# Genie-Kim/PintheMemory

Measured on AMD Instinct MI355X. Metric: train imgs/sec 768x768 bs=8 R50-DeepLabV3+ +mem, higher is better.
Workload: dtype f32

## Files before the change

### include/pinmem_hip.h

```cpp
#ifndef PINMEM_HIP_H
#define PINMEM_HIP_H
#include <stddef.h>
#include <stdint.h>

#ifdef __cplusplus
extern "C" {
#endif

typedef enum pm_status { PM_OK = 0, PM_EINVAL = -1, PM_EWORKSPACE = -2, PM_ELAUNCH = -3, PM_EUNSUPPORTED = -4 } pm_status;

typedef enum pm_dtype { PM_F32 = 0, PM_BF16 = 1 } pm_dtype;
#define PM_TF_ZERO_PAD64 1

typedef struct pm_tensor {
  void* ptr;
  int32_t n, h, w, c;
  int64_t pitch;
  int32_t dtype;
  int32_t flags;
} pm_tensor;

#define PM_ABI_VERSION 460

typedef struct pm_conv_params {
  int32_t struct_size;
  int32_t kh, kw, stride, pad, dil;
  int32_t prec;
  void* wino_v;
  int64_t wino_v_bytes;
  void* wxf;
  int64_t wxf_bytes;
  int32_t wxf_valid;
} pm_conv_params;

typedef struct pm_conv_epilogue {
  int64_t struct_size;
  const float* bias;
  const float* scale;
  const float* shift;
  const float* residual;
  int64_t residual_pitch;
  int32_t relu;
  float* bn_partials;
  int64_t bn_partials_bytes;
} pm_conv_epilogue;

const char* pm_last_error(void);
int pm_version(void);

size_t pm_conv_workspace(const pm_tensor* x, const pm_tensor* y, const pm_conv_params* p, int which );
size_t pm_conv_winograd_v_bytes(const pm_tensor* x, const pm_tensor* y, const pm_conv_params* p);
size_t pm_conv_wxf_bytes(const pm_tensor* x, const pm_tensor* y, const pm_conv_params* p);
size_t pm_conv_wxf_bytes_dgrad(const pm_tensor* dy, const pm_tensor* dx, const pm_conv_params* p);
typedef struct pm_wxf_job {
  const float* w;
  void* wxf;
  int64_t wxf_bytes;
  int32_t cout, kh, kw, cin;
  int32_t dgrad;
  int32_t reserved;
} pm_wxf_job;
int pm_conv_wxf_refresh_bf16(const pm_wxf_job* jobs, int n, void* stream);
int pm_conv_wxf_refresh_f32(const pm_wxf_job* jobs, int n, void* stream);
size_t pm_conv_bn_partials_bytes(const pm_tensor* x, const pm_tensor* y, const pm_conv_params* p);
int pm_conv_fwd(const pm_tensor* x, const float* w_krsc, const pm_tensor* y, const pm_conv_params* p,
                const pm_conv_epilogue* ep, void* ws, size_t ws_bytes, void* stream);
int pm_conv_bwd_data(const pm_tensor* dy, const float* w_krsc, const pm_tensor* dx, const pm_conv_params* p,
                     const pm_tensor* add, void* ws, size_t ws_bytes, void* stream);
int pm_conv_bwd_data_masked(const pm_tensor* dy, const float* w_krsc, const pm_tensor* dx, const pm_conv_params* p,
                            const pm_tensor* add, const uint8_t* add_mask, void* ws, size_t ws_bytes, void* stream);
int pm_conv_bwd_weight(const pm_tensor* x, const pm_tensor* dy, float* dw_krsc, float* dbias, const pm_conv_params* p,
                       void* ws, size_t ws_bytes, void* stream);

typedef struct pm_routing {
  int32_t struct_size;
  int32_t winograd;
  int32_t winograd_fused;
  int32_t conv16;
  int32_t conv16_wide;
  int32_t conv16_persistent;
  int32_t wgrad16;
  int32_t bf16_wgrad;
  int32_t split;
} pm_routing;
int pm_routing_get(pm_routing* out);
int pm_routing_set(const pm_routing* r);


int pm_set_winograd(int mode);
int pm_set_winograd_fused(int on);
int pm_set_conv16(int on);
int pm_set_bf16_wgrad(int on);
int pm_set_wgrad16(int on);
int pm_set_split(int on);

int pm_profile_enable(int on);
int pm_profile_dump(const char* csv_path);
int pm_profile_read(int mode, int bm, int bn, int km, int nst, double* total_ms, double* total_flops, int64_t* launches, int clear);
int pm_profile_read_prec(int mode, int bm, int bn, int km, int nst, int prec, double* total_ms, double* total_flops, int64_t* launches, int clear);
int pm_profile_read_bytes(int mode, int bm, int bn, int km, int nst, int prec, double* total_bytes);

size_t pm_bn_workspace(const pm_tensor* x);
int pm_bn_stats(const pm_tensor* x, float* moments, void* ws, size_t ws_bytes, void* stream);
int pm_bn_stats_finalize(const pm_tensor* x, float eps, float* mean, float* invstd, float* running_mean , float* running_var ,
                         float momentum, void* ws, size_t ws_bytes, void* stream);
int pm_bn_merge(const float* parts, int world, int c, float* moments, void* stream);
int pm_bn_merge_finalize(const float* parts, int world, int c, float eps, float* mean, float* invstd, float* running_mean ,
                         float* running_var , float momentum, void* stream);
int pm_bn_finalize(const float* moments, int c, float eps, float* mean, float* invstd,
                   float* running_mean, float* running_var, float momentum, void* stream);
int pm_bn_apply(const pm_tensor* x, const float* mean, const float* invstd, const float* gamma, const float* beta,
                const pm_tensor* residual , int relu, const pm_tensor* y, void* stream);
int pm_bn_apply_mask(const pm_tensor* x, const float* mean, const float* invstd, const float* gamma, const float* beta,
                     const pm_tensor* residual , int relu, const pm_tensor* y, uint8_t* mask , void* stream);
int pm_bn_bwd_reduce_mask(const pm_tensor* dy, const uint8_t* mask, const pm_tensor* x, const float* mean, const float* invstd,
                          const pm_tensor* gmask , float* sums, void* ws, size_t ws_bytes, void* stream);
int pm_bn_apply_mask_affine(const pm_tensor* x, const float* mean, const float* invstd, const float* gamma, const float* beta,
                            const pm_tensor* r, const float* r_mean, const float* r_invstd, const float* r_gamma, const float* r_beta,
                            int relu, const pm_tensor* y, uint8_t* mask , void* stream);
int pm_bn_bwd_apply_mask(const pm_tensor* dy, const uint8_t* mask, const pm_tensor* x, const float* mean, const float* invstd, const float* gamma,
                         const float* sums, float count, const pm_tensor* dx, void* stream);
int pm_bn_bwd_reduce(const pm_tensor* dy, const pm_tensor* y , const pm_tensor* x, const float* mean, const float* invstd,
                     const float* gamma , const float* beta , int relu, const pm_tensor* gmask ,
                     float* sums, void* ws, size_t ws_bytes, void* stream);
int pm_bn_bwd_apply(const pm_tensor* dy, const pm_tensor* y , const pm_tensor* x, const float* mean, const float* invstd,
                    const float* gamma, const float* beta , const float* sums, float count, int relu, const pm_tensor* dx,
                    const pm_tensor* dres , void* stream);
int pm_bn_partials_finalize(const float* partials, int64_t pixels, int c, float eps, float* mean, float* invstd, float* running_mean ,
                            float* running_var , float momentum, float* moments , void* stream);
int pm_bn_fold(const float* gamma, const float* beta, const float* running_mean, const float* running_var, const float* conv_bias,
               int c, float eps, float* scale, float* shift, void* stream);
int pm_bn_fold_multi(const void* table, const int* cs, const int* offs, int n, int max_c, int total, float eps, float* arena, void* stream);
int pm_relu_bwd(const pm_tensor* dy, const pm_tensor* y, const pm_tensor* dx, void* stream);
int pm_add(const pm_tensor* a, const pm_tensor* b, const pm_tensor* y, void* stream);
int pm_add_n(const pm_tensor* const* xs, int n, const pm_tensor* y, void* stream);
int pm_copy(const pm_tensor* src, const pm_tensor* dst, void* stream);
int pm_scale_shift_act(const pm_tensor* x, const float* scale, const float* shift, const pm_tensor* residual, int relu,
                       const pm_tensor* y, void* stream);

size_t pm_instnorm_workspace(int n, int h, int w, int c);
int pm_instnorm_fwd(const void* x, void* y, int n, int h, int w, int c, int64_t x_pitch, int64_t y_pitch, int dtype, const float* gamma ,
                    const float* beta , float eps, int relu, float* mean, float* invstd, void* ws, size_t ws_bytes, void* stream);
int pm_instnorm_bwd(const void* dy, const void* x, const void* y , void* dx, int n, int h, int w, int c, int64_t dy_pitch, int64_t x_pitch, int64_t y_pitch,
                    int64_t dx_pitch, int dtype, const float* gamma , const float* mean, const float* invstd, int relu, float* dgamma ,
                    float* dbeta , void* ws, size_t ws_bytes, void* stream);

int pm_cast(const pm_tensor* x, const pm_tensor* y, void* stream);

int pm_maxpool3x3s2_fwd(const pm_tensor* x, const pm_tensor* y, uint8_t* argmax, void* stream);
int pm_maxpool3x3s2_bwd(const pm_tensor* dy, const uint8_t* argmax, const pm_tensor* dx, void* stream);
int pm_maxpool3x3s2_bn_relu_fwd(const pm_tensor* x, const float* mean, const float* invstd, const float* gamma, const float* beta, const pm_tensor* y,
                                uint8_t* argmax, void* stream);
int pm_bn_bwd_reduce_pool(const pm_tensor* dy_pooled, const uint8_t* argmax, const pm_tensor* x, const float* mean, const float* invstd, const float* gamma,
                          const float* beta, float* sums, void* ws, size_t ws_bytes, void* stream);
int pm_bn_bwd_apply_pool(const pm_tensor* dy_pooled, const uint8_t* argmax, const pm_tensor* x, const float* mean, const float* invstd, const float* gamma,
// ... 176 lines not shown
```

### pinthememory_amd/csrc/conv_igemm.hip

```cpp
#include <stdlib.h>
#include <algorithm>
#include <type_traits>
#include <vector>

#include "pm_common.h"

#include "conv_igemm_kernel.h"

namespace {

template <int ZL, bool O16 = false>
__global__ __launch_bounds__(256) void splitk_reduce_vec_kernel(const float* __restrict__ ws, int ksplit, long slab, int M, int Nn,
                                                                float* __restrict__ C, long c_pitch, const float* bias,
                                                                const float* scale, const float* shift, const float* residual,
                                                                long res_pitch, int relu, const unsigned char* res_mask) {
  constexpr int GP = 256 / ZL;
  __shared__ float4 red[ZL > 1 ? ZL : 1][GP];
  const int gl = threadIdx.x % GP, zl = threadIdx.x / GP;
  const long groups = (long)M * Nn / 4;
  for (long g0 = (long)blockIdx.x * GP; g0 < groups; g0 += (long)gridDim.x * GP) {
    const long grp = g0 + gl;
    float4 v = make_float4(0.f, 0.f, 0.f, 0.f);
    if (grp < groups)
#pragma unroll 8
// ... 401 lines not shown
    return launch<MODE>(k, pl, st, 1, flops);
  });
}

int check_common(const pm_tensor* x, const pm_tensor* y, const pm_conv_params* p) {
  PM_REQUIRE(x && y && p && x->ptr && y->ptr, PM_EINVAL, "conv: null tensor");
  PM_REQUIRE(p->struct_size == (int32_t)sizeof(pm_conv_params), PM_EINVAL, "conv: pm_conv_params.struct_size %d != %zu -- caller built against another pinmem_hip.h (library ABI %d)",
             p->struct_size, sizeof(pm_conv_params), PM_ABI_VERSION);
  PM_REQUIRE(p->kh >= 1 && p->kw >= 1 && p->dil >= 1 && p->pad >= 0, PM_EINVAL, "conv: bad geometry");
  PM_REQUIRE(p->stride == 1 || p->stride == 2, PM_EUNSUPPORTED, "conv: stride %d unsupported (1 or 2)", p->stride);
  const int ho = (x->h + 2 * p->pad - p->dil * (p->kh - 1) - 1) / p->stride + 1;
  const int wo = (x->w + 2 * p->pad - p->dil * (p->kw - 1) - 1) / p->stride + 1;
  PM_REQUIRE(ho == y->h && wo == y->w && x->n == y->n, PM_EINVAL, "conv: output %dx%d does not match geometry (%dx%d)", y->h, y->w, ho, wo);
  PM_REQUIRE((x->dtype == PM_F32 || x->dtype == PM_BF16) && (y->dtype == PM_F32 || y->dtype == PM_BF16), PM_EUNSUPPORTED, "conv: dtype %d / %d", x->dtype, y->dtype);
  for (const pm_tensor* t : {x, y}) {
    if (pm_is_bf16(t)) PM_REQUIRE(pm_vec8(t), PM_EINVAL, "conv: bf16 tensors must be 16B aligned with pitch %% 8 == 0 and channels %% 8 == 0");
    else PM_REQUIRE(pm_vec_ok(t), PM_EINVAL, "conv: tensors must be 16B aligned with pitch %% 4 == 0");
  }
  PM_REQUIRE(x->c % 4 == 0, PM_EUNSUPPORTED, "conv: Cin %% 4 != 0 unsupported (pad the input channels)");
  PM_REQUIRE((y->c % 4 == 0) || (p->kh * p->kw == 1), PM_EUNSUPPORTED, "conv: Cout %% 4 != 0 only for 1x1");
  PM_REQUIRE(x->pitch >= x->c && y->pitch >= y->c, PM_EINVAL, "conv: pitch < channels");
  PM_REQUIRE(pm_pixels(x) * x->pitch < (1ll << 29) && pm_pixels(y) * y->pitch < (1ll << 29) && (int64_t)y->c * x->c * p->kh * p->kw < (1ll << 29),
             PM_EUNSUPPORTED, "conv: tensor too large for 32-bit byte offsets (2 GiB per tensor)");
  return PM_OK;
}

void fill_geom(ConvK& k, const pm_tensor* x, const pm_tensor* y, const pm_conv_params* p) {
  k.N = x->n, k.H = x->h, k.W = x->w, k.Cin = x->c, k.x_pitch = x->pitch;
  k.Ho = y->h, k.Wo = y->w, k.Cout = y->c, k.y_pitch = y->pitch;
  k.kh = p->kh, k.kw = p->kw, k.stride = p->stride, k.pad = p->pad, k.dil = p->dil;
  k.sshift = p->stride == 2 ? 1 : 0;
  k.prec = p->prec != 0 ? 1 : 0;
  k.T_eff = p->kh * p->kw, k.tk_w = p->kw, k.ky0 = k.kx0 = 0, k.ksy = k.ksx = 1;
  k.sub = k.sub_cy = k.sub_cx = 0, k.Hc = x->h, k.Wc = x->w;
  k.bias = k.scale = k.shift = k.residual = nullptr;
  k.res_pitch = 0, k.res_mask = nullptr, k.relu = 0, k.stats = nullptr, k.io16 = 0;
  k.stage_ep = 1;
  k.spl_prio = 1;
  k.n_group = 8;
  k.batch_xcd = 0;
  k.a_bs = k.b_bs = k.c_bs = 0;
}

struct WinoPlan {
  bool use;
  pm_wino_geom g;
  int Kp, P;
  size_t v_bytes, m_bytes, u_bytes;
  Plan pl;
};
inline bool wino_wgrad_pays(int cin, int cout) { return (long)cin * cout >= 256 * 256; }
WinoPlan wino_plan(const pm_tensor* xin, int cout, const pm_conv_params* p, bool wgrad = false) {
  WinoPlan wp{};
  if (wgrad && !wino_wgrad_pays(xin->c, cout)) return wp;
  if (pm_route.winograd == 0 || p->kh != 3 || p->kw != 3 || p->stride != 1 || p->pad != p->dil || p->prec != 0) return wp;
  const int cin = xin->c;
  if (cin < 128 || cout < 128 || (cout & 3) || (cin & 3)) return wp;
  int m = 0;
  double best_ratio = 0.6;
  for (int cand = pm_route.winograd; cand >= 2; cand -= 2) {
    const pm_wino_geom g = pm_wino_make_geom(xin->n, xin->h, xin->w, p->dil, cand);
    const double cover = (double)(cand * g.TY * p->dil) * (double)(cand * g.TX * p->dil) / ((double)xin->h * xin->w);
    const double ratio = cover * (cand + 2) * (cand + 2) / (9.0 * cand * cand);
    if (ratio <= best_ratio) best_ratio = ratio, m = cand, wp.g = g;
  }
  if (!m) return wp;
  wp.P = (m + 2) * (m + 2);
  wp.Kp = (cin + BK - 1) / BK * BK;
  if (wp.g.tiles * (long)std::max(wp.Kp, cout) * 4 >= (1ll << 31)) return wp;
  wp.v_bytes = pm_align_up((size_t)wp.P * wp.g.tiles * wp.Kp * sizeof(float), 256);
  wp.m_bytes = pm_align_up((size_t)wp.P * wp.g.tiles * cout * sizeof(float), 256);
  wp.u_bytes = pm_align_up((size_t)wp.P * cout * wp.Kp * sizeof(float), 256);
  wp.pl.bm = 128, wp.pl.bn = 128;
  if (pm_cdiv(cout, 128) * 128 > cout * 1.12 && pm_cdiv(cout, 64) * 64 < pm_cdiv(cout, 128) * 128) wp.pl.bn = 64;
  if (wp.g.tiles <= 4608 && !pm_route.split) wp.pl.bm = 64;
  wp.pl.tiles_m = pm_cdiv(wp.g.tiles, wp.pl.bm), wp.pl.tiles_n = pm_cdiv(cout, wp.pl.bn);
  wp.pl.ksplit = 1, wp.pl.kper = wp.Kp, wp.pl.ws_bytes = 0;
  wp.use = true;
  return wp;
}
inline size_t wino_ws(const WinoPlan& wp) { return wp.v_bytes + wp.m_bytes + wp.u_bytes; }

int wino_conv(const pm_tensor* xin, const float* w, int w_cout, int w_cin, bool dgrad, const pm_tensor* yout, const WinoPlan& wp,
              const pm_conv_epilogue& ep, void* ws, hipStream_t st, float* v_keep = nullptr, float* u_ext = nullptr, bool u_valid = false) {
  float* V = v_keep ? v_keep : (float*)ws;
  float* Mo = (float*)((char*)ws + wp.v_bytes);
  float* U = u_ext ? u_ext : (float*)((char*)ws + wp.v_bytes + wp.m_bytes);
  const int cout = yout->c;
  if (int e = pm_wino_input_xf((const float*)xin->ptr, xin->pitch, xin->c, wp.Kp, wp.g, V, st)) return e;
  if (!(u_ext && u_valid))
    if (int e = pm_wino_filter_xf(w, w_cout, w_cin, wp.Kp, dgrad, wp.g.m, U, st)) return e;
  const pm_tensor xv = {V, 1, 1, (int32_t)wp.g.tiles, wp.Kp, wp.Kp};
  const pm_tensor yv = {Mo, 1, 1, (int32_t)wp.g.tiles, cout, cout};
  const pm_conv_params p1 = {(int32_t)sizeof(pm_conv_params), 1, 1, 1, 0, 1, 0};
  ConvK k;
  fill_geom(k, &xv, &yv, &p1);
  k.A = V, k.B = U, k.C = Mo;
  k.M = (int)wp.g.tiles, k.Nn = cout, k.K = wp.Kp;
  k.a_bytes = (unsigned)(wp.g.tiles * wp.Kp * 4), k.b_bytes = (unsigned)((long)cout * wp.Kp * 4), k.kmode = K_FAST;
  k.c_pitch = cout, k.c_split = 0;
  k.a_bs = wp.g.tiles * wp.Kp, k.b_bs = (long)cout * wp.Kp, k.c_bs = wp.g.tiles * cout;
  if (pm_route.winograd_fused && wp.g.m == 4 && wp.Kp % 16 == 0) {
    ProfScope prof(st, 3, 32, 32, 0, 0, 1, wp.g.tiles, cout, wp.Kp, wp.P, 1, 2.0 * wp.P * (double)wp.g.tiles * cout * xin->c);
    const int e = pm_wino_fused_f4(V, U, cout, wp.Kp, wp.g, (float*)yout->ptr, yout->pitch, ep.bias, ep.scale, ep.shift, ep.residual, ep.residual_pitch, ep.relu, st);
    prof.done();
    return e;
  }
  if (int e = launch<MODE_FWD>(k, wp.pl, st, wp.P, 2.0 * wp.P * (double)wp.g.tiles * cout * xin->c)) return e;
  return pm_wino_output_xf(Mo, cout, wp.g, (float*)yout->ptr, yout->pitch, ep.bias, ep.scale, ep.shift, ep.residual, ep.residual_pitch, ep.relu, st);
}

struct WinoWgradPlan {
  Plan pl;
  size_t slab_bytes;
};
WinoWgradPlan wino_wgrad_plan(const WinoPlan& wp, int cout) {
  WinoWgradPlan q{};
  q.pl.bm = 128, q.pl.bn = 128;
  if (pm_cdiv(wp.Kp, 128) * 128 > wp.Kp * 1.12 && pm_cdiv(wp.Kp, 64) * 64 < pm_cdiv(wp.Kp, 128) * 128) q.pl.bn = 64;
  q.pl.tiles_m = pm_cdiv(cout, 128), q.pl.tiles_n = pm_cdiv(wp.Kp, q.pl.bn);
  const long ksteps = (wp.g.tiles + BK - 1) / BK;
  const long per_split = (long)q.pl.tiles_m * q.pl.tiles_n * wp.P;
  long ks = std::max<long>(1, std::min<long>((768 + per_split / 2) / per_split, ksteps / 8));
  const long steps_per = (ksteps + ks - 1) / ks;
  ks = (ksteps + steps_per - 1) / steps_per;
  q.pl.ksplit = (int)ks, q.pl.kper = (int)(steps_per * BK), q.pl.ws_bytes = 0;
  q.slab_bytes = pm_align_up((size_t)ks * wp.P * cout * wp.Kp * sizeof(float), 256);
  return q;
}
inline size_t wino_wgrad_ws(const WinoPlan& wp, const WinoWgradPlan& q) { return wp.v_bytes + wp.m_bytes + q.slab_bytes; }

int wino_wgrad(const pm_tensor* x, const pm_tensor* dy, float* dw, const WinoPlan& wp, const WinoWgradPlan& q, void* ws, hipStream_t st,
               float* v_kept = nullptr) {
  float* V = v_kept ? v_kept : (float*)ws;
  float* Z = (float*)((char*)ws + wp.v_bytes);
  float* slab = (float*)((char*)ws + wp.v_bytes + wp.m_bytes);
  const int cout = dy->c;
  if (!v_kept)
    if (int e = pm_wino_input_xf((const float*)x->ptr, x->pitch, x->c, wp.Kp, wp.g, V, st)) return e;
  if (int e = pm_wino_dy_xf((const float*)dy->ptr, dy->pitch, cout, wp.g, Z, st)) return e;
  const pm_tensor xv = {V, 1, 1, (int32_t)wp.g.tiles, wp.Kp, wp.Kp};
  const pm_tensor zv = {Z, 1, 1, (int32_t)wp.g.tiles, cout, cout};
  const pm_conv_params p1 = {(int32_t)sizeof(pm_conv_params), 1, 1, 1, 0, 1, 0};
  ConvK k;
  fill_geom(k, &xv, &zv, &p1);
  k.A = Z, k.B = V, k.C = slab;
  k.M = cout, k.Nn = wp.Kp, k.K = (int)wp.g.tiles;
  k.a_bytes = (unsigned)(wp.g.tiles * cout * 4), k.b_bytes = (unsigned)(wp.g.tiles * wp.Kp * 4), k.kmode = K_MID;
  k.c_pitch = wp.Kp, k.c_split = (long)wp.P * cout * wp.Kp;
  k.a_bs = wp.g.tiles * cout, k.b_bs = wp.g.tiles * wp.Kp, k.c_bs = (long)cout * wp.Kp;
  if (int e = launch<MODE_WGRAD>(k, q.pl, st, wp.P, 2.0 * wp.P * (double)wp.g.tiles * cout * x->c)) return e;
  return pm_wino_dw_xf(slab, q.pl.ksplit, cout, x->c, wp.Kp, wp.g.m, dw, st);
}

struct Bf16Plan {
  bool use;
  bool c16;
  pm_conv16 k16;
  bool inplace;
  int Cp;
  long M, Nn, Kf;
  size_t xb_bytes, wb_bytes;
  Plan pl;
};
Bf16Plan bf16_plan(const pm_tensor* xin, const pm_tensor* yout, const pm_conv_params* p) {
  Bf16Plan b{};
  if ((p->prec != 2 && !pm_is_bf16(xin) && !pm_is_bf16(yout)) || xin->c < 32) return b;
  b.Cp = (xin->c + 63) / 64 * 64;
  const long T = (long)p->kh * p->kw;
  b.M = pm_pixels(yout), b.Nn = yout->c, b.Kf = T * b.Cp / 2;
  b.inplace = pm_is_bf16(xin) && (xin->c % 64 == 0 || ((xin->flags & PM_TF_ZERO_PAD64) && xin->pitch >= b.Cp));
  const size_t xb = b.inplace ? (size_t)pm_pixels(xin) * xin->pitch * 2 : (size_t)pm_pixels(xin) * b.Cp * 2, wb = (size_t)yout->c * T * b.Cp * 2;
  if (xb >= (1ull << 31) || wb >= (1ull << 31)) return b;
  b.xb_bytes = b.inplace ? 0 : pm_align_up(xb, 256), b.wb_bytes = pm_align_up(wb, 256);
  b.pl = make_plan(MODE_FWD, b.M, b.Nn, b.Kf, true);
  if (b.pl.bn < 64) return b;
  b.use = true;
  constexpr long C16_MIN_M = 256;
  b.c16 = false;
  if (pm_route.conv16 && b.M >= C16_MIN_M && p->stride >= 1) {
    pm_conv16& k = b.k16;
    k = pm_conv16{};
    k.N = xin->n, k.H = xin->h, k.W = xin->w, k.Ho = yout->h, k.Wo = yout->w;
    k.a_pitch = b.inplace ? xin->pitch : b.Cp, k.Cp = b.Cp;
    k.kh = p->kh, k.kw = p->kw, k.stride = p->stride, k.pad = p->pad, k.dil = p->dil;
    k.M = (int)b.M, k.Nn = (int)b.Nn, k.K = (int)(T * b.Cp), k.ksteps = k.K / 64;
    k.c_pitch = yout->pitch, k.c_f32 = pm_is_bf16(yout) ? 0 : 1;
    pm_conv16_plan(&k);
    b.c16 = pm_route.conv16 == 2 || k.wide || k.bm == 64 || k.ksteps_per == 1 || (b.pl.bm == 64 && k.ksteps >= 16);
  }
  return b;
}
inline size_t bf16_ws(const Bf16Plan& b) {
  return b.xb_bytes + b.wb_bytes + std::max(pm_align_up(b.pl.ws_bytes, 256), b.c16 ? pm_conv16_slab_bytes(&b.k16) : (size_t)0);
}

int conv_bf16(const pm_tensor* xin, const float* w, int w_cout, int w_cin, bool rotate, const pm_tensor* yout, const pm_conv_params* pe, const Bf16Plan& b,
              const pm_conv_epilogue& e0, void* ws, hipStream_t st, char* wb_ext = nullptr, bool wb_valid = false) {
  char* xb = b.inplace ? (char*)xin->ptr : (char*)ws;
  char* wb = wb_ext ? wb_ext : (char*)ws + b.xb_bytes;
  float* slab = (float*)((char*)ws + b.xb_bytes + b.wb_bytes);
  const int T = pe->kh * pe->kw;
  if (!b.inplace) {
    if (pm_is_bf16(xin)) {
      if (int e = pm16_pad_rows((const pm_bf16*)xin->ptr, xin->pitch, xin->c, b.Cp, pm_pixels(xin), (pm_bf16*)xb, st)) return e;
    } else if (int e = pm_bf16_cast_rows((const float*)xin->ptr, xin->pitch, xin->c, b.Cp, pm_pixels(xin), xb, st)) return e;
  }
  if (!(wb_ext && wb_valid))
    if (int e = pm_bf16_cast_weights(w, w_cout, T, w_cin, b.Cp, rotate, wb, st)) return e;
  const long xpitch16 = b.inplace ? xin->pitch : b.Cp;
  if (b.c16) {
    const bool o16 = pm_is_bf16(yout);
    const bool ok = (!e0.bn_partials || o16) &&
                    (o16 ? ((yout->c | yout->pitch | (e0.residual ? e0.residual_pitch : 0)) & 7) == 0 && pm_aligned16(yout->ptr) && pm_aligned16(e0.residual)
                         : !(e0.scale || e0.residual || e0.relu));
    if (ok) {
      pm_conv16 k = b.k16;
      k.A = (const pm_bf16*)xb, k.B = (const pm_bf16*)wb;
      const double fl = 2.0 * (double)b.M * (double)b.Nn * (double)T * (double)xin->c * (g_prof_on ? pm_conv16_executed_fraction(&k) : 1.0);
      ProfScope prof(st, k.wide ? 5 : 4, k.bm, k.bn, pm_conv16w_persistent(&k), 5, k.wide ? 3 : (k.ksteps_per == 1 ? 1 : 2), k.M, k.Nn, k.K / 2, 1, k.ksplit, fl);
      return run_planned(k.ksplit, b.M, b.Nn, slab, (float*)yout->ptr, (long)yout->pitch, e0, o16, nullptr, st, [&](float* C, bool slabs) {
        k.C = C;
        if (!slabs) set_epilogue(k, e0), k.stats = o16 ? e0.bn_partials : nullptr;
// ... 407 lines not shown
}
extern "C" int pm_set_split(int on) {
  pm_route.split = on ? 1 : 0;
  return PM_OK;
}
extern "C" int pm_set_bf16_wgrad(int on) {
  pm_route.bf16_wgrad = on != 0;
  return PM_OK;
}
extern "C" int pm_profile_enable(int on) {
  g_prof_on = on != 0;
  return PM_OK;
}
extern "C" int pm_profile_read_prec(int mode, int bm, int bn, int km, int nst, int prec, double* total_ms, double* total_flops, int64_t* launches, int clear);
extern "C" int pm_profile_read(int mode, int bm, int bn, int km, int nst, double* total_ms, double* total_flops, int64_t* launches, int clear) {
  return pm_profile_read_prec(mode, bm, bn, km, nst, -1, total_ms, total_flops, launches, clear);
}
extern "C" int pm_profile_read_prec(int mode, int bm, int bn, int km, int nst, int prec, double* total_ms, double* total_flops, int64_t* launches, int clear) {
  double ms = 0.0, fl = 0.0;
  int64_t n = 0;
  for (const ProfRec& r : g_prof) {
    if ((mode >= 0 && r.mode != mode) || (bm >= 0 && r.bm != bm) || (bn >= 0 && r.bn != bn) || (km >= 0 && r.km != km) || (nst >= 0 && r.nst != nst) ||
        (prec >= 0 && r.prec != prec))
      continue;
    float t = 0.f;
    if (hipEventSynchronize(r.b) != hipSuccess || hipEventElapsedTime(&t, r.a, r.b) != hipSuccess) continue;
    ms += t, fl += r.flops, ++n;
  }
  if (clear) {
    for (const ProfRec& r : g_prof) (void)hipEventDestroy(r.a), (void)hipEventDestroy(r.b);
    g_prof.clear();
  }
  if (total_ms) *total_ms = ms;
  if (total_flops) *total_flops = fl;
  if (launches) *launches = n;
  return PM_OK;
}

extern "C" int pm_profile_read_bytes(int mode, int bm, int bn, int km, int nst, int prec, double* total_bytes) {
  double b = 0.0;
  for (const ProfRec& r : g_prof) {
    if ((mode >= 0 && r.mode != mode) || (bm >= 0 && r.bm != bm) || (bn >= 0 && r.bn != bn) || (km >= 0 && r.km != km) || (nst >= 0 && r.nst != nst) ||
        (prec >= 0 && r.prec != prec))
      continue;
    b += r.bytes;
  }
  if (total_bytes) *total_bytes = b;
  return PM_OK;
}

extern "C" int pm_profile_dump(const char* path) {
  PM_REQUIRE(path, PM_EINVAL, "pm_profile_dump: null path");
  FILE* f = fopen(path, "w");
  PM_REQUIRE(f, PM_EINVAL, "pm_profile_dump: cannot open %s", path);
  fprintf(f, "mode,bm,bn,km,nst,prec,M,N,K,batch,ksplit,ms,gflop\n");
  for (const ProfRec& r : g_prof) {
    float t = 0.f;
    if (hipEventSynchronize(r.b) != hipSuccess || hipEventElapsedTime(&t, r.a, r.b) != hipSuccess) continue;
    fprintf(f, "%d,%d,%d,%d,%d,%d,%d,%d,%d,%d,%d,%.5f,%.4f\n", r.mode, r.bm, r.bn, r.km, r.nst, r.prec, r.M, r.Nn, r.K, r.batch, r.ksplit, t, r.flops * 1e-9);
  }
  fclose(f);
  return PM_OK;
}

extern "C" size_t pm_conv_workspace(const pm_tensor* x, const pm_tensor* y, const pm_conv_params* p0, int which) {
  const pm_conv_params tp = tier_params(p0, x, y);
  return route_conv(which, x, y, &tp).ws_bytes;
}
extern "C" size_t pm_conv_winograd_v_bytes(const pm_tensor* x, const pm_tensor* y, const pm_conv_params* p0) {
  if (!x || !y || !p0) return 0;
  const pm_conv_params tp = tier_params(p0, x, y);
  return route_conv(MODE_FWD, x, y, &tp).v_keep_bytes;
}
extern "C" size_t pm_conv_wxf_bytes(const pm_tensor* x, const pm_tensor* y, const pm_conv_params* p0) {
  if (!x || !y || !p0) return 0;
  const pm_conv_params tp = tier_params(p0, x, y);
  return route_conv(MODE_FWD, x, y, &tp).wxf_bytes;
}
extern "C" size_t pm_conv_wxf_bytes_dgrad(const pm_tensor* dy, const pm_tensor* dx, const pm_conv_params* p0) {
  if (!dy || !dx || !p0) return 0;
  const pm_conv_params tp = tier_params(p0, dy, dx);
  return route_conv(MODE_DGRAD, dx, dy, &tp).wxf_bytes;
}
extern "C" size_t pm_conv_bn_partials_bytes(const pm_tensor* x, const pm_tensor* y, const pm_conv_params* p0) {
  if (!x || !y || !p0 || check_common(x, y, p0) != PM_OK) return 0;
  const pm_conv_params tp = tier_params(p0, x, y);
  return route_conv(MODE_FWD, x, y, &tp).bn_bytes;
}

extern "C" int pm_conv_wxf_refresh_f32(const pm_wxf_job* jobs, int n, void* stream) {
  PM_REQUIRE(n >= 0 && (jobs || n == 0), PM_EINVAL, "conv_wxf_refresh_f32: bad job table");
  std::vector<const float*> w(n);
  std::vector<float*> U(n);
  std::vector<int> cout(n), cin(n), kp(n), m(n);
  for (int i = 0; i < n; ++i) {
    const pm_wxf_job& q = jobs[i];
    PM_REQUIRE(q.w && q.wxf && q.cout > 0 && q.cin > 0 && q.kh == 3 && q.kw == 3 && q.dgrad == 0, PM_EINVAL,
               "conv_wxf_refresh_f32: job %d: forward transforms of 3x3 filters only", i);
    PM_REQUIRE(pm_aligned16(q.wxf), PM_EINVAL, "conv_wxf_refresh_f32: job %d: buffer must be 16-byte aligned", i);
    const int Kp = (q.cin + BK - 1) / BK * BK;
    const size_t u4 = pm_align_up((size_t)36 * q.cout * Kp * sizeof(float), 256), u2 = pm_align_up((size_t)16 * q.cout * Kp * sizeof(float), 256);
    PM_REQUIRE((size_t)q.wxf_bytes == u4 || (size_t)q.wxf_bytes == u2, PM_EINVAL, "conv_wxf_refresh_f32: job %d: %ld bytes is neither the F(4x4) nor the F(2x2) transform of %d x %d",
               i, (long)q.wxf_bytes, q.cout, q.cin);
    w[i] = q.w, U[i] = (float*)q.wxf, cout[i] = q.cout, cin[i] = q.cin, kp[i] = Kp, m[i] = (size_t)q.wxf_bytes == u4 ? 4 : 2;
  }
  return pm_wino_filter_xf_multi(w.data(), U.data(), cout.data(), cin.data(), kp.data(), m.data(), n, (hipStream_t)stream);
}

extern "C" int pm_conv_fwd(const pm_tensor* x, const float* w, const pm_tensor* y, const pm_conv_params* p0,
                           const pm_conv_epilogue* ep, void* ws, size_t ws_bytes, void* stream) {
  if (int e = check_common(x, y, p0)) return e;
  const pm_conv_params tp = tier_params(p0, x, y);
  const pm_conv_params* p = &tp;
  PM_REQUIRE(!ep || ep->struct_size == (int64_t)sizeof(pm_conv_epilogue), PM_EINVAL,
             "conv_fwd: pm_conv_epilogue.struct_size %ld != %zu -- caller built against another pinmem_hip.h (library ABI %d)", ep ? (long)ep->struct_size : 0l,
             sizeof(pm_conv_epilogue), PM_ABI_VERSION);
  PM_REQUIRE(w && pm_aligned16(w), PM_EINVAL, "conv_fwd: weight null or unaligned");
  pm_conv_epilogue e0 = {(int64_t)sizeof(pm_conv_epilogue), nullptr, nullptr, nullptr, nullptr, 0, 0};
  if (ep) e0 = *ep;
  PM_REQUIRE((e0.scale == nullptr) == (e0.shift == nullptr), PM_EINVAL, "conv_fwd: scale and shift go together");
  const ConvRoute r = route_conv(MODE_FWD, x, y, p);
  if (e0.bn_partials) {
    PM_REQUIRE(!e0.relu && !e0.residual, PM_EINVAL, "conv_fwd: bn_partials are the statistics of the convolution output (no residual / ReLU)");
    PM_REQUIRE(r.bn_bytes != 0 && (size_t)e0.bn_partials_bytes >= r.bn_bytes, PM_EINVAL, "conv_fwd: this call cannot emit bn_partials (ask pm_conv_bn_partials_bytes): %zu needed", r.bn_bytes);
  }
  PM_REQUIRE(ws_bytes >= r.ws_bytes && (ws || r.ws_bytes == 0), PM_EWORKSPACE, "conv_fwd: workspace %zu < %zu", ws_bytes, r.ws_bytes);
  hipStream_t st = (hipStream_t)stream;
  switch (r.kind) {
    case R_WINO: {
      float* keep = (p->wino_v && (size_t)p->wino_v_bytes >= r.wino.v_bytes) ? (float*)p->wino_v : nullptr;
      float* uext = (p->wxf && (size_t)p->wxf_bytes >= r.wino.u_bytes) ? (float*)p->wxf : nullptr;
      return wino_conv(x, w, y->c, x->c, false, y, r.wino, e0, ws, st, keep, uext, p->wxf_valid != 0);
    }
    case R_BF16: {
      char* wext = (p->wxf && (size_t)p->wxf_bytes >= r.b16.wb_bytes) ? (char*)p->wxf : nullptr;
      return conv_bf16(x, w, y->c, x->c, false, y, &r.pe, r.b16, e0, ws, st, wext, p->wxf_valid != 0);
    }
    default:
      PM_REQUIRE(pm_is_f32(x), PM_EUNSUPPORTED, "conv_fwd: a bf16 input needs at least 32 channels (got %d)", x->c);
      return conv_direct<MODE_FWD>(x, y, w, p, r.pl, e0, ws, st);
  }
}

extern "C" int pm_conv_bwd_data(const pm_tensor* dy, const float* w, const pm_tensor* dx, const pm_conv_params* p0, const pm_tensor* add,
                                void* ws, size_t ws_bytes, void* stream) {
  return pm_conv_bwd_data_masked(dy, w, dx, p0, add, nullptr, ws, ws_bytes, stream);
}

extern "C" int pm_conv_bwd_data_masked(const pm_tensor* dy, const float* w, const pm_tensor* dx, const pm_conv_params* p0, const pm_tensor* add,
                                       const uint8_t* add_mask, void* ws, size_t ws_bytes, void* stream) {
  if (int e = check_common(dx, dy, p0)) return e;
  const pm_conv_params tp = tier_params(p0, dy, dx);
  const pm_conv_params* p = &tp;
  PM_REQUIRE(!add || (add->ptr && pm_same_shape(add, dx) && add->dtype == dx->dtype), PM_EINVAL, "conv_bwd_data: `add` must match dx (shape and dtype)");
  PM_REQUIRE(!add || !pm_is_bf16(add) || pm_vec8(add), PM_EINVAL, "conv_bwd_data: bf16 `add` must be 16B aligned with pitch %% 8 == 0");
  PM_REQUIRE(w && pm_aligned16(w), PM_EINVAL, "conv_bwd_data: weight null or unaligned");
  const ConvRoute r = route_conv(MODE_DGRAD, dx, dy, p);
  PM_REQUIRE(ws_bytes >= r.ws_bytes && (ws || r.ws_bytes == 0), PM_EWORKSPACE, "conv_bwd_data: workspace %zu < %zu", ws_bytes, r.ws_bytes);
  if (add_mask) {
    PM_REQUIRE(add && pm_is_f32(add) && pm_is_f32(dy) && pm_vec4(add) && pm_vec4(dx), PM_EINVAL, "conv_bwd_data: a masked `add` is an fp32 tensor with 16-byte rows and c %% 4 == 0");
    PM_REQUIRE(r.kind == R_DIRECT, PM_EUNSUPPORTED,
               "conv_bwd_data: a masked `add` is served by the fp32 implicit-GEMM route only (this call routes to %s)",
               r.kind == R_WINO ? "Winograd" : (r.kind == R_BF16 ? "the bf16 kernels" : "the stride-2 class kernels"));
  }
  hipStream_t st = (hipStream_t)stream;
  const pm_conv_epilogue e1 = {(int64_t)sizeof(pm_conv_epilogue), nullptr, nullptr, nullptr, add ? (const float*)add->ptr : nullptr, add ? add->pitch : 0, 0};
  switch (r.kind) {
    case R_S2_NATIVE: return dgrad_s2_bf16(dy, w, dx, p, add, r.s2n, ws, st);
    case R_S2_PARITY: return dgrad_s2_parity(dy, w, dx, p, add, r, ws, st);
    case R_BF16: {
      char* wext = (p->wxf && (size_t)p->wxf_bytes >= r.b16.wb_bytes) ? (char*)p->wxf : nullptr;
      return conv_bf16(dy, w, dy->c, dx->c, true, dx, &r.pe, r.b16, e1, ws, st, wext, p->wxf_valid != 0);
    }
    case R_WINO: return wino_conv(dy, w, dy->c, dx->c, true, dx, r.wino, e1, ws, st);
    default:
      PM_REQUIRE(pm_is_f32(dy), PM_EUNSUPPORTED, "conv_bwd_data: a bf16 dy needs at least 32 channels and a stride-1 geometry the forward form covers");
      return conv_direct<MODE_DGRAD>(dx, dy, w, p, r.pl, e1, ws, st, add_mask);
  }
}

extern "C" int pm_conv_bwd_weight(const pm_tensor* x0, const pm_tensor* dy0, float* dw, float* dbias, const pm_conv_params* p0, void* ws,
                                  size_t ws_bytes, void* stream) {
  if (int e = check_common(x0, dy0, p0)) return e;
  const pm_conv_params tp = tier_params(p0, x0, dy0);
  const pm_conv_params* p = &tp;
  PM_REQUIRE(dw && pm_aligned16(dw), PM_EINVAL, "conv_bwd_weight: dw null or unaligned");
  const ConvRoute r = route_conv(MODE_WGRAD, x0, dy0, p);
  PM_REQUIRE(ws && ws_bytes >= r.ws_bytes, PM_EWORKSPACE, "conv_bwd_weight: workspace %zu < %zu", ws_bytes, r.ws_bytes);
  hipStream_t st = (hipStream_t)stream;
  const pm_tensor *x = x0, *dy = dy0;
  pm_tensor x32, dy32;
  if (!r.native16 && pm_is_bf16(x0)) {
    if (int e = upcast(x0, (char*)ws + r.x32_off, &x32, st)) return e;
    x = &x32;
  }
  if (pm_is_bf16(dy0) && (!r.native16 || dbias)) {
    if (int e = upcast(dy0, (char*)ws + r.dy32_off, &dy32, st)) return e;
    if (!r.native16) dy = &dy32;
  }
  int e;
  switch (r.kind) {
    case R_BF16_WGRAD: e = conv_wgrad_bf16(x, dy, dw, p, r.b16w, ws, st); break;
    case R_WINO_WGRAD: e = wino_wgrad(x, dy, dw, r.wino, r.wino_w, ws, st, (p->wino_v && (size_t)p->wino_v_bytes >= r.wino.v_bytes) ? (float*)p->wino_v : nullptr); break;
    default: e = conv_wgrad_direct(x, dy, dw, p, r, ws, st);
  }
  if (e || !dbias) return e;
  const pm_tensor* dyb = pm_is_bf16(dy0) ? &dy32 : dy0;
  const long P = pm_pixels(dyb);
  const int rpb = colsum_rows(P, dyb->c), nb = pm_cdiv(P, rpb);
  float* part = (float*)((char*)ws + r.bias_off);
  if (dyb->pitch == ((dyb->c + 3) & ~3) && dyb->pitch <= 64 && pm_aligned16(dyb->ptr))
    hipLaunchKernelGGL(colsum_partial_narrow_kernel, dim3(nb), dim3(256), 0, st, (const float*)dyb->ptr, (int)(dyb->pitch / 4), P, dyb->c, rpb, part);
  else
    hipLaunchKernelGGL(colsum_partial_kernel, dim3(nb, pm_cdiv(dyb->c, 64)), dim3(256), 0, st, (const float*)dyb->ptr, (long)dyb->pitch, P, dyb->c, rpb, part);
  hipLaunchKernelGGL(colsum_final_kernel, dim3(pm_cdiv(dyb->c, 64)), dim3(1024), 0, st, (const float*)part, nb, dyb->c, dbias);
  return pm_check_launch("conv_bias_grad");
}
```

### pinthememory_amd/csrc/pm_common.h

```cpp
#pragma once
#include <hip/hip_runtime.h>
#include <algorithm>
#include <atomic>
#include <stdarg.h>
#include <stdint.h>
#include <stdio.h>

#include "../../include/pinmem_hip.h"

void pm_set_error(const char* fmt, ...);

#define PM_REQUIRE(cond, code, ...)      \
  do {                                   \
    if (!(cond)) {                       \
      pm_set_error(__VA_ARGS__);         \
      return (code);                     \
    }                                    \
  } while (0)

static inline int pm_check_launch(const char* what) {
  hipError_t e = hipGetLastError();
  if (e != hipSuccess) {
    pm_set_error("%s: launch failed: %s", what, hipGetErrorString(e));
    return PM_ELAUNCH;
  }
  return PM_OK;
}

static inline bool pm_aligned16(const void* p) { return (reinterpret_cast<uintptr_t>(p) & 15u) == 0; }
static inline int64_t pm_pixels(const pm_tensor* t) { return (int64_t)t->n * t->h * t->w; }
static inline int pm_cdiv(int64_t a, int64_t b) { return (int)((a + b - 1) / b); }
static inline size_t pm_align_up(size_t v, size_t a) { return (v + a - 1) / a * a; }

static inline bool pm_vec_ok(const pm_tensor* t) { return pm_aligned16(t->ptr) && (t->pitch % 4) == 0; }
static inline bool pm_is_f32(const pm_tensor* t) { return t->dtype == PM_F32; }
static inline bool pm_is_bf16(const pm_tensor* t) { return t->dtype == PM_BF16; }
#define PM_REQUIRE_F32(t, who) PM_REQUIRE(!(t) || pm_is_f32(t), PM_EUNSUPPORTED, "%s: fp32 tensors only (got dtype %d)", who, (t)->dtype)
static inline bool pm_vec8(const pm_tensor* t) { return pm_is_bf16(t) && pm_aligned16(t->ptr) && (t->pitch % 8) == 0 && (t->c % 8) == 0; }

struct pm_wino_geom {
  int N, H, W, d, m, TY, TX;
  long tiles;
};
pm_wino_geom pm_wino_make_geom(int n, int h, int w, int d, int m);
int pm_wino_input_xf(const float* x, long pitch, int C, int Kp, const pm_wino_geom& g, float* V, hipStream_t st);
int pm_wino_filter_xf(const float* w, int Cout, int Cin, int Kp, bool dgrad, int m, float* U, hipStream_t st);
int pm_wino_filter_xf_multi(const float* const* w, float* const* U, const int* cout, const int* cin, const int* kp, const int* m, int n, hipStream_t st);
int pm_wino_output_xf(const float* M, int Cout, const pm_wino_geom& g, float* y, long ypitch, const float* bias, const float* scale, const float* shift,
                      const float* residual, long res_pitch, int relu, hipStream_t st);
int pm_wino_fused_f4(const float* V, const float* U, int Cout, int Kp, const pm_wino_geom& g, float* y, long ypitch, const float* bias, const float* scale,
                     const float* shift, const float* residual, long res_pitch, int relu, hipStream_t st);
int pm_wino_dy_xf(const float* dy, long pitch, int Cout, const pm_wino_geom& g, float* Z, hipStream_t st);
int pm_wino_dw_xf(const float* slab, int ks, int Cout, int Cin, int Kp, int m, float* dw, hipStream_t st);

int pm_bf16_cast_rows(const float* x, long pitch, int C, int Cp, long P, void* out, hipStream_t st);
int pm_bf16_cast_weights(const float* w, int Cout, int T, int Cin, int Cp, bool rotate, void* out, hipStream_t st);
struct PmS2Classes {
  int ky0[4], nky[4], kx0[4], nkx[4];
  void* out[4];
};
int pm_bf16_cast_weights_s2(const float* w, int Cout, int kh, int kw, int Cin, int Cp, const PmS2Classes* cl, hipStream_t st);
int pm_bf16_transpose_taps(const float* x, long pitch, int C, int N, int H, int W, int Ho, int Wo, int kh, int kw, int stride, int pad, int dil, void* out,
                           hipStream_t st);

typedef unsigned short pm_bf16;
int pm16_to_f32(const pm_bf16* x, long pitch, int C, long P, float* out, long out_pitch, hipStream_t st);
int pm16_pad_rows(const pm_bf16* x, long pitch, int C, int Cp, long P, pm_bf16* out, hipStream_t st);

struct pm_conv16 {
  const pm_bf16* A;
  const pm_bf16* B;
  void* C;
  int N, H, W, Ho, Wo;
  long a_pitch;
  int Cp;
  int kh, kw, stride, pad, dil;
  int M, Nn, K, ksteps;
  long c_pitch;
  int c_f32;
  const float *bias, *scale, *shift;
  const void* residual;
  long res_pitch;
  int relu;
  float* stats;
  int bm, bn, tiles_m, tiles_n, ksplit, ksteps_per;
  long c_split;
  int wide;
};
void pm_conv16_plan(pm_conv16* k);
int pm_conv16w_launch(const pm_conv16* k, hipStream_t st);
int pm_conv16w_persistent(const pm_conv16* k);
size_t pm_conv16_slab_bytes(const pm_conv16* k);
double pm_conv16_executed_fraction(const pm_conv16* k);
int pm_conv16_launch(const pm_conv16* k, hipStream_t st);

struct pm_wgrad16 {
  const pm_bf16* X;
  const pm_bf16* DY;
  float* C;
  int N, H, W, Ho, Wo;
  long x_pitch, dy_pitch;
  int Cin, Cout, kh, kw, stride, pad, dil;
  int M, Nn, P;
  int kper, ksplit;
  long c_split;
  int bm, bn, tiles_m, tiles_n;
};
bool pm_wgrad16_plan(pm_wgrad16* k);
int pm_wgrad16_launch(const pm_wgrad16* k, hipStream_t st);

struct pm_gemm_pw {
  const float* A;
  const float* B;
  float* C;
  const float *bias, *scale, *shift, *residual;
  const unsigned char* res_mask;
  long a_pitch, c_pitch, res_pitch;
  int b_sn, b_sk;
  long M;
  int Nn, K, relu;
};
bool pm_pwstream_ok(const pm_gemm_pw* g);
int pm_pwstream_launch(const pm_gemm_pw* g, hipStream_t st);

constexpr int PM_MAX_DEVICES = 64;
inline int pm_device_cus(int dev) {
  static std::atomic<int> cached[PM_MAX_DEVICES];
  const bool keep = dev >= 0 && dev < PM_MAX_DEVICES;
// ... 307 lines not shown
```

### pinthememory_amd/csrc/winograd.hip

```cpp
#include "pm_common.h"

namespace {

enum { W_BT = 0, W_AT = 1, W_G = 2, W_A = 3, W_GT = 4 };

template <int MT>
__host__ __device__ constexpr float wino_bt(int i, int j) {
  if (MT == 2) {
    constexpr float t[4][4] = {{1, 0, -1, 0}, {0, 1, 1, 0}, {0, -1, 1, 0}, {0, 1, 0, -1}};
    return t[i & 3][j & 3];
  }
  constexpr float t[6][6] = {{4, 0, -5, 0, 1, 0}, {0, -4, -4, 1, 1, 0}, {0, 4, -4, -1, 1, 0}, {0, -2, -1, 2, 1, 0}, {0, 2, -1, -2, 1, 0}, {0, 4, 0, -5, 0, 1}};
  return t[i][j];
}
template <int MT>
__host__ __device__ constexpr float wino_at(int i, int j) {
  if (MT == 2) {
    constexpr float t[2][4] = {{1, 1, 1, 0}, {0, 1, -1, -1}};
    return t[i & 1][j & 3];
  }
  constexpr float t[4][6] = {{1, 1, 1, 1, 1, 0}, {0, 1, -1, 2, -2, 0}, {0, 1, 1, 4, 4, 0}, {0, 1, -1, 8, -8, 1}};
  return t[i][j];
}
template <int MT>
// ... 2 lines not shown
    constexpr float t[4][3] = {{1, 0, 0}, {0.5f, 0.5f, 0.5f}, {0.5f, -0.5f, 0.5f}, {0, 0, 1}};
    return t[i & 3][j];
  }
  constexpr float t[6][3] = {{1.f / 4, 0, 0},          {-1.f / 6, -1.f / 6, -1.f / 6}, {-1.f / 6, 1.f / 6, -1.f / 6},
                             {1.f / 24, 1.f / 12, 1.f / 6}, {1.f / 24, -1.f / 12, 1.f / 6},  {0, 0, 1}};
  return t[i][j];
}
template <int MT, int WHICH>
__host__ __device__ constexpr float wino_coef(int r, int c) {
  return WHICH == W_BT ? wino_bt<MT>(r, c) : WHICH == W_AT ? wino_at<MT>(r, c) : WHICH == W_G ? wino_g<MT>(r, c) : WHICH == W_A ? wino_at<MT>(c, r) : wino_g<MT>(c, r);
}

template <int W>
struct Vec {
  float v[W];
};
template <int W>
__device__ __forceinline__ Vec<W> vzero() {
  Vec<W> r;
#pragma unroll
  for (int i = 0; i < W; ++i) r.v[i] = 0.f;
  return r;
}
template <int W>
__device__ __forceinline__ Vec<W> vload(const float* p) {
  Vec<W> r;
  if constexpr (W == 4) {
    const float4 q = PM_LD4(p);
    r.v[0] = q.x, r.v[1] = q.y, r.v[2] = q.z, r.v[3] = q.w;
  } else if constexpr (W == 2) {
    const float2 q = *reinterpret_cast<const float2*>(p);
    r.v[0] = q.x, r.v[1] = q.y;
  } else {
    r.v[0] = *p;
  }
  return r;
}
template <int W>
__device__ __forceinline__ void vstore(float* p, const Vec<W>& r) {
  if constexpr (W == 4) PM_ST4(p, make_float4(r.v[0], r.v[1], r.v[2], r.v[3]));
  else if constexpr (W == 2) *reinterpret_cast<float2*>(p) = make_float2(r.v[0], r.v[1]);
  else *p = r.v[0];
}

template <int MT, int WHICH, int R, int C, int W>
__device__ __forceinline__ void mat_apply(const Vec<W> (&in)[C], Vec<W> (&out)[R]) {
#pragma unroll
  for (int r = 0; r < R; ++r) {
    Vec<W> acc = vzero<W>();
    bool first = true;
#pragma unroll
    for (int c = 0; c < C; ++c) {
      const float k = wino_coef<MT, WHICH>(r, c);
      if (k == 0.f) continue;
#pragma unroll
      for (int i = 0; i < W; ++i) {
        if (first) acc.v[i] = k == 1.f ? in[c].v[i] : (k == -1.f ? -in[c].v[i] : k * in[c].v[i]);
        else if (k == 1.f) acc.v[i] += in[c].v[i];
        else if (k == -1.f) acc.v[i] -= in[c].v[i];
        else acc.v[i] = fmaf(k, in[c].v[i], acc.v[i]);
      }
      first = false;
    }
    out[r] = acc;
  }
}

struct TileId {
  int n, ry, rx, ty, tx;
};
__device__ __forceinline__ TileId decode_tile(unsigned tile, const pm_wino_geom& g) {
  TileId t;
  t.tx = (int)(tile % (unsigned)g.TX);
  unsigned q = tile / (unsigned)g.TX;
  t.ty = (int)(q % (unsigned)g.TY);
  q /= (unsigned)g.TY;
  t.rx = (int)(q % (unsigned)g.d);
  q /= (unsigned)g.d;
  t.ry = (int)(q % (unsigned)g.d);
  t.n = (int)(q / (unsigned)g.d);
  return t;
}

template <int MT, int W>
__global__ __launch_bounds__(256) void wino_input_kernel(const float* __restrict__ x, long xp, int C, int Kp, const pm_wino_geom g, float* __restrict__ V) {
  constexpr int A = MT + 2;
  const unsigned kg = Kp / W;
  const unsigned total = (unsigned)g.tiles * kg;
  const long plane = g.tiles * (long)Kp;
  for (unsigned i = blockIdx.x * 256u + threadIdx.x; i < total; i += gridDim.x * 256u) {
    const unsigned tile = i / kg;
    const int c = (int)(i - tile * kg) * W;
    const TileId t = decode_tile(tile, g);
    const bool cok = c < C;
    Vec<W> tt[A][A];
#pragma unroll
    for (int b = 0; b < A; ++b) {
      const int xx = t.rx + g.d * (MT * t.tx + b - 1);
      const bool xok = cok && (unsigned)xx < (unsigned)g.W;
      Vec<W> col[A], o[A];
#pragma unroll
      for (int a = 0; a < A; ++a) {
        const int yy = t.ry + g.d * (MT * t.ty + a - 1);
        col[a] = (xok && (unsigned)yy < (unsigned)g.H) ? vload<W>(x + ((long)(t.n * g.H + yy) * g.W + xx) * xp + c) : vzero<W>();
      }
      mat_apply<MT, W_BT>(col, o);
#pragma unroll
      for (int a = 0; a < A; ++a) tt[a][b] = o[a];
    }
    float* out = V + (long)tile * Kp + c;
#pragma unroll
    for (int a = 0; a < A; ++a) {
      Vec<W> o[A];
      mat_apply<MT, W_BT>(tt[a], o);
#pragma unroll
      for (int b = 0; b < A; ++b) vstore<W>(out + (a * A + b) * plane, o[b]);
    }
  }
}

template <int MT, int W>
__global__ __launch_bounds__(256) void wino_output_kernel(const float* __restrict__ M, int Cout, const pm_wino_geom g, float* __restrict__ y, long yp,
                                                          const float* __restrict__ bias, const float* __restrict__ scale,
                                                          const float* __restrict__ shift, const float* __restrict__ residual, long rp, int relu) {
  constexpr int A = MT + 2;
  const unsigned cg = Cout / W;
  const unsigned total = (unsigned)g.tiles * cg;
  const long plane = g.tiles * (long)Cout;
  for (unsigned i = blockIdx.x * 256u + threadIdx.x; i < total; i += gridDim.x * 256u) {
    const unsigned tile = i / cg;
    const int c = (int)(i - tile * cg) * W;
    const TileId t = decode_tile(tile, g);
    const float* in = M + (long)tile * Cout + c;
    Vec<W> s[MT][A];
#pragma unroll
    for (int b = 0; b < A; ++b) {
      Vec<W> col[A], o[MT];
#pragma unroll
      for (int a = 0; a < A; ++a) col[a] = vload<W>(in + (a * A + b) * plane);
      mat_apply<MT, W_AT>(col, o);
#pragma unroll
      for (int a = 0; a < MT; ++a) s[a][b] = o[a];
    }
    Vec<W> bi = vzero<W>(), sc = vzero<W>(), sh = vzero<W>();
    if (bias) bi = vload<W>(bias + c);
    if (scale) sc = vload<W>(scale + c), sh = vload<W>(shift + c);
#pragma unroll
    for (int a = 0; a < MT; ++a) {
      const int yy = t.ry + g.d * (MT * t.ty + a);
      Vec<W> o[MT];
      mat_apply<MT, W_AT>(s[a], o);
#pragma unroll
      for (int b = 0; b < MT; ++b) {
        const int xx = t.rx + g.d * (MT * t.tx + b);
        if (yy >= g.H || xx >= g.W) continue;
        const long pix = (long)(t.n * g.H + yy) * g.W + xx;
        Vec<W> v = o[b];
        if (bias) {
#pragma unroll
          for (int q = 0; q < W; ++q) v.v[q] += bi.v[q];
        }
        if (scale) {
#pragma unroll
          for (int q = 0; q < W; ++q) v.v[q] = v.v[q] * sc.v[q] + sh.v[q];
        }
        if (residual) {
          const Vec<W> rr = vload<W>(residual + pix * rp + c);
#pragma unroll
          for (int q = 0; q < W; ++q) v.v[q] += rr.v[q];
        }
        if (relu) {
#pragma unroll
          for (int q = 0; q < W; ++q) v.v[q] = fmaxf(v.v[q], 0.f);
        }
        vstore<W>(y + pix * yp + c, v);
      }
    }
  }
}

template <int MT, bool DGRAD>
__device__ __forceinline__ void wino_filter_block(const float* __restrict__ w, int Cout, int Cin, int Kp, float* __restrict__ U, int bx, int by,
                                                  float (*sg)[32][33]) {
  constexpr int A = MT + 2;
  const int tx = threadIdx.x & 31, ty = threadIdx.x >> 5;
  const int R = DGRAD ? Cin : Cout;
  const int Kr = DGRAD ? Cout : Cin;
// ... 16 lines not shown
    Vec<4> col[3], o[A];
#pragma unroll
    for (int ky = 0; ky < 3; ++ky)
#pragma unroll
      for (int e = 0; e < 4; ++e) col[ky].v[e] = DGRAD ? sg[(2 - ky) * 3 + (2 - kx)][4 * q + e][j] : sg[ky * 3 + kx][j][4 * q + e];
    mat_apply<MT, W_G>(col, o);
#pragma unroll
    for (int a = 0; a < A; ++a) gg[a][kx] = o[a];
  }
  float* out = U + (long)row * Kp + k;
#pragma unroll
  for (int a = 0; a < A; ++a) {
    Vec<4> o[A];
    mat_apply<MT, W_G>(gg[a], o);
#pragma unroll
    for (int b = 0; b < A; ++b) {
#pragma unroll
      for (int e = 0; e < 4; ++e)
        if (k + e >= Kr) o[b].v[e] = 0.f;
      vstore<4>(out + (a * A + b) * plane, o[b]);
    }
  }
}
template <int MT, bool DGRAD>
__global__ __launch_bounds__(256) void wino_filter_kernel(const float* __restrict__ w, int Cout, int Cin, int Kp, float* __restrict__ U) {
  __shared__ float sg[9][32][33];
  wino_filter_block<MT, DGRAD>(w, Cout, Cin, Kp, U, blockIdx.x, blockIdx.y, sg);
}

constexpr int WR_BATCH = 48;
struct WinoRefreshJobs {
  const float* w[WR_BATCH];
  float* U[WR_BATCH];
  int cout[WR_BATCH], cin[WR_BATCH], kp[WR_BATCH], m[WR_BATCH];
  int start[WR_BATCH + 1];
  int n;
};
__global__ __launch_bounds__(256) void wino_filter_multi_kernel(const WinoRefreshJobs t) {
  __shared__ float sg[9][32][33];
  int j = 0;
  while (j + 1 < t.n && (int)blockIdx.x >= t.start[j + 1]) ++j;
  const int local = (int)blockIdx.x - t.start[j];
  const int nbx = t.kp[j] / 32;
  const int bx = local % nbx, by = local / nbx;
  if (t.m[j] == 4) wino_filter_block<4, false>(t.w[j], t.cout[j], t.cin[j], t.kp[j], t.U[j], bx, by, sg);
  else wino_filter_block<2, false>(t.w[j], t.cout[j], t.cin[j], t.kp[j], t.U[j], bx, by, sg);
}

template <int MT, int W>
__global__ __launch_bounds__(256) void wino_dy_kernel(const float* __restrict__ dy, long yp, int Cout, const pm_wino_geom g, float* __restrict__ Z) {
  constexpr int A = MT + 2;
  const unsigned cg = Cout / W;
  const unsigned total = (unsigned)g.tiles * cg;
  const long plane = g.tiles * (long)Cout;
  for (unsigned i = blockIdx.x * 256u + threadIdx.x; i < total; i += gridDim.x * 256u) {
    const unsigned tile = i / cg;
    const int c = (int)(i - tile * cg) * W;
    const TileId t = decode_tile(tile, g);
    Vec<W> r[A][MT];
#pragma unroll
    for (int b = 0; b < MT; ++b) {
      const int xx = t.rx + g.d * (MT * t.tx + b);
      Vec<W> col[MT], o[A];
#pragma unroll
      for (int a = 0; a < MT; ++a) {
        const int yy = t.ry + g.d * (MT * t.ty + a);
        col[a] = (yy < g.H && xx < g.W) ? vload<W>(dy + ((long)(t.n * g.H + yy) * g.W + xx) * yp + c) : vzero<W>();
      }
      mat_apply<MT, W_A>(col, o);
#pragma unroll
      for (int a = 0; a < A; ++a) r[a][b] = o[a];
    }
    float* out = Z + (long)tile * Cout + c;
#pragma unroll
    for (int a = 0; a < A; ++a) {
      Vec<W> o[A];
      mat_apply<MT, W_A>(r[a], o);
#pragma unroll
      for (int b = 0; b < A; ++b) vstore<W>(out + (a * A + b) * plane, o[b]);
    }
  }
}

template <int MT>
__global__ __launch_bounds__(256) void wino_dw_kernel(const float* __restrict__ slab, int ks, int Cout, int Cin, int Kp, float* __restrict__ dw) {
  constexpr int A = MT + 2, P = A * A;
  const long total = (long)Cout * Cin, plane = (long)Cout * Kp;
  for (long i = (long)blockIdx.x * 256 + threadIdx.x; i < total; i += (long)gridDim.x * 256) {
    const int co = (int)(i / Cin), ci = (int)(i - (long)co * Cin);
    const float* in = slab + (long)co * Kp + ci;
    float du[P];
#pragma unroll
    for (int q = 0; q < P; ++q) du[q] = 0.f;
    for (int z = 0; z < ks; ++z) {
      float ld[P];
#pragma unroll
      for (int q = 0; q < P; ++q) ld[q] = in[((long)z * P + q) * plane];
#pragma unroll
      for (int q = 0; q < P; ++q) du[q] += ld[q];
    }
    Vec<1> h[3][A];
#pragma unroll
    for (int b = 0; b < A; ++b) {
      Vec<1> col[A], o[3];
#pragma unroll
      for (int a = 0; a < A; ++a) col[a].v[0] = du[a * A + b];
      mat_apply<MT, W_GT>(col, o);
#pragma unroll
      for (int k = 0; k < 3; ++k) h[k][b] = o[k];
    }
    float* out = dw + (long)co * 9 * Cin + ci;
#pragma unroll
    for (int k = 0; k < 3; ++k) {
      Vec<1> o[3];
      mat_apply<MT, W_GT>(h[k], o);
#pragma unroll
      for (int l = 0; l < 3; ++l) out[(k * 3 + l) * (long)Cin] = o[l].v[0];
    }
  }
}

typedef float f32x16 __attribute__((ext_vector_type(16)));

struct WinoFusedArgs {
  const float* V;
  const float* U;
  float* y;
  long yp;
  int Cout, Kp;
  pm_wino_geom g;
  const float* bias;
  const float* scale;
  const float* shift;
  const float* residual;
  long rp;
  int relu;
  int ncb;
};

constexpr int WF_THREADS = 768, WF_TB = 32, WF_CB = 32, WF_BK = 16, WF_P = 36;
constexpr size_t WF_LDS = (size_t)WF_P * WF_TB * (WF_CB + 1) * sizeof(float);

__global__ __launch_bounds__(WF_THREADS) void wino_fused_f4_kernel(const WinoFusedArgs a) {
  extern __shared__ __align__(16) float4 lds4[];
  const int tid = threadIdx.x, lane = tid & 63, wave = tid >> 6;
  const int lid = pm_xcd_remap(blockIdx.x, gridDim.x);
  const int tb = lid / a.ncb, cb = lid - tb * a.ncb;
  const long tile0 = (long)tb * WF_TB;
  const int co0 = cb * WF_CB;

  const int rem = tid & 255, row = rem >> 2, chunk = rem & 3, pgrp = tid >> 8;
  const bool is_a = row < WF_TB;
  bool valid;
  const float* gp;
  long plane;
  if (is_a) {
    const long tile = tile0 + row;
    valid = tile < a.g.tiles;
    gp = a.V + (valid ? tile : 0) * a.Kp + chunk * 4;
    plane = a.g.tiles * (long)a.Kp;
  } else {
    const int co = co0 + row - WF_TB;
    valid = co < a.Cout;
    gp = a.U + (long)(valid ? co : 0) * a.Kp + chunk * 4;
    plane = (long)a.Cout * a.Kp;
  }
// ... 29 lines not shown
      acc[j] = __builtin_amdgcn_mfma_f32_32x32x2f32(a0.z, b0.z, acc[j], 0, 0, 0);
      acc[j] = __builtin_amdgcn_mfma_f32_32x32x2f32(a0.w, b0.w, acc[j], 0, 0, 0);
      acc[j] = __builtin_amdgcn_mfma_f32_32x32x2f32(a1.x, b1.x, acc[j], 0, 0, 0);
      acc[j] = __builtin_amdgcn_mfma_f32_32x32x2f32(a1.y, b1.y, acc[j], 0, 0, 0);
      acc[j] = __builtin_amdgcn_mfma_f32_32x32x2f32(a1.z, b1.z, acc[j], 0, 0, 0);
      acc[j] = __builtin_amdgcn_mfma_f32_32x32x2f32(a1.w, b1.w, acc[j], 0, 0, 0);
    }
  };

  const int nk = a.Kp / WF_BK;
  gload(0);
  lstore();
  __syncthreads();
  for (int kt = 0; kt < nk; ++kt) {
    if (kt + 1 < nk) gload((kt + 1) * WF_BK);
    compute();
    __syncthreads();
    if (kt + 1 < nk) {
      lstore();
      __syncthreads();
    }
  }

  float* Ms = reinterpret_cast<float*>(lds4);
#pragma unroll
  for (int j = 0; j < 3; ++j) {
    const int pnt = wave * 3 + j;
#pragma unroll
    for (int q = 0; q < 16; ++q) Ms[(pnt * WF_TB + (q & 3) + 8 * (q >> 2) + 4 * half) * (WF_CB + 1) + l31] = acc[j][q];
  }
  __syncthreads();
  constexpr int MT = 4, A = 6;
  for (int idx = tid; idx < WF_TB * WF_CB; idx += WF_THREADS) {
    const int t = idx >> 5, c = idx & 31;
    const long tile = tile0 + t;
    const int co = co0 + c;
    if (tile >= a.g.tiles || co >= a.Cout) continue;
    const TileId ti = decode_tile((unsigned)tile, a.g);
    Vec<1> sv[MT][A];
#pragma unroll
    for (int b = 0; b < A; ++b) {
      Vec<1> col[A], o[MT];
#pragma unroll
      for (int aa = 0; aa < A; ++aa) col[aa].v[0] = Ms[((aa * A + b) * WF_TB + t) * (WF_CB + 1) + c];
      mat_apply<MT, W_AT>(col, o);
#pragma unroll
      for (int aa = 0; aa < MT; ++aa) sv[aa][b] = o[aa];
    }
    const float bi = a.bias ? a.bias[co] : 0.f, sc = a.scale ? a.scale[co] : 0.f, sh = a.scale ? a.shift[co] : 0.f;
#pragma unroll
    for (int aa = 0; aa < MT; ++aa) {
      const int yy = ti.ry + a.g.d * (MT * ti.ty + aa);
      Vec<1> o[MT];
      mat_apply<MT, W_AT>(sv[aa], o);
#pragma unroll
      for (int b = 0; b < MT; ++b) {
        const int xx = ti.rx + a.g.d * (MT * ti.tx + b);
        if (yy >= a.g.H || xx >= a.g.W) continue;
        const long pix = (long)(ti.n * a.g.H + yy) * a.g.W + xx;
        float v = o[b].v[0];
        if (a.bias) v += bi;
        if (a.scale) v = v * sc + sh;
        if (a.residual) v += a.residual[pix * a.rp + co];
        if (a.relu) v = fmaxf(v, 0.f);
        a.y[pix * a.yp + co] = v;
      }
    }
  }
}

inline unsigned nblocks(long total) { return (unsigned)std::min<long>((total + 255) / 256, 1 << 20); }

}

pm_wino_geom pm_wino_make_geom(int n, int h, int w, int d, int m) {
  pm_wino_geom g;
  g.N = n, g.H = h, g.W = w, g.d = d, g.m = m;
  g.TY = (pm_cdiv(h, d) + m - 1) / m, g.TX = (pm_cdiv(w, d) + m - 1) / m;
  g.tiles = (long)n * d * d * g.TY * g.TX;
  return g;
}

int pm_wino_input_xf(const float* x, long pitch, int C, int Kp, const pm_wino_geom& g, float* V, hipStream_t st) {
  if (g.m == 4) hipLaunchKernelGGL((wino_input_kernel<4, 2>), dim3(nblocks(g.tiles * (Kp / 2))), dim3(256), 0, st, x, pitch, C, Kp, g, V);
  else hipLaunchKernelGGL((wino_input_kernel<2, 4>), dim3(nblocks(g.tiles * (Kp / 4))), dim3(256), 0, st, x, pitch, C, Kp, g, V);
  return pm_check_launch("wino_input");
}

int pm_wino_filter_xf(const float* w, int Cout, int Cin, int Kp, bool dgrad, int m, float* U, hipStream_t st) {
  const int R = dgrad ? Cin : Cout;
  dim3 grid(Kp / 32, pm_cdiv(R, 32));
  if (m == 4) {
    if (dgrad) hipLaunchKernelGGL((wino_filter_kernel<4, true>), grid, dim3(256), 0, st, w, Cout, Cin, Kp, U);
    else hipLaunchKernelGGL((wino_filter_kernel<4, false>), grid, dim3(256), 0, st, w, Cout, Cin, Kp, U);
  } else {
    if (dgrad) hipLaunchKernelGGL((wino_filter_kernel<2, true>), grid, dim3(256), 0, st, w, Cout, Cin, Kp, U);
    else hipLaunchKernelGGL((wino_filter_kernel<2, false>), grid, dim3(256), 0, st, w, Cout, Cin, Kp, U);
  }
  return pm_check_launch("wino_filter");
}

int pm_wino_filter_xf_multi(const float* const* w, float* const* U, const int* cout, const int* cin, const int* kp, const int* m, int n, hipStream_t st) {
  for (int i0 = 0; i0 < n; i0 += WR_BATCH) {
    WinoRefreshJobs t;
    t.n = std::min(WR_BATCH, n - i0);
    long blocks = 0;
    for (int i = 0; i < t.n; ++i) {
      t.w[i] = w[i0 + i], t.U[i] = U[i0 + i], t.cout[i] = cout[i0 + i], t.cin[i] = cin[i0 + i], t.kp[i] = kp[i0 + i], t.m[i] = m[i0 + i];
      t.start[i] = (int)blocks;
      blocks += (long)(kp[i0 + i] / 32) * pm_cdiv(cout[i0 + i], 32);
    }
    t.start[t.n] = (int)blocks;
    if (blocks == 0) continue;
    hipLaunchKernelGGL(wino_filter_multi_kernel, dim3((unsigned)blocks), dim3(256), 0, st, t);
    if (int e = pm_check_launch("wino_filter_multi")) return e;
  }
  return PM_OK;
}

int pm_wino_output_xf(const float* M, int Cout, const pm_wino_geom& g, float* y, long ypitch, const float* bias, const float* scale, const float* shift,
                      const float* residual, long res_pitch, int relu, hipStream_t st) {
  if (g.m == 4)
    hipLaunchKernelGGL((wino_output_kernel<4, 2>), dim3(nblocks(g.tiles * (Cout / 2))), dim3(256), 0, st, M, Cout, g, y, ypitch, bias, scale, shift, residual,
                       res_pitch, relu);
  else
    hipLaunchKernelGGL((wino_output_kernel<2, 4>), dim3(nblocks(g.tiles * (Cout / 4))), dim3(256), 0, st, M, Cout, g, y, ypitch, bias, scale, shift, residual,
                       res_pitch, relu);
  return pm_check_launch("wino_output");
}

int pm_wino_dy_xf(const float* dy, long pitch, int Cout, const pm_wino_geom& g, float* Z, hipStream_t st) {
  if (g.m == 4) hipLaunchKernelGGL((wino_dy_kernel<4, 2>), dim3(nblocks(g.tiles * (Cout / 2))), dim3(256), 0, st, dy, pitch, Cout, g, Z);
  else hipLaunchKernelGGL((wino_dy_kernel<2, 4>), dim3(nblocks(g.tiles * (Cout / 4))), dim3(256), 0, st, dy, pitch, Cout, g, Z);
  return pm_check_launch("wino_dy");
}

int pm_wino_dw_xf(const float* slab, int ks, int Cout, int Cin, int Kp, int m, float* dw, hipStream_t st) {
  const unsigned nb = (unsigned)std::min<long>(((long)Cout * Cin + 255) / 256, 1 << 16);
  if (m == 4) hipLaunchKernelGGL(wino_dw_kernel<4>, dim3(nb), dim3(256), 0, st, slab, ks, Cout, Cin, Kp, dw);
  else hipLaunchKernelGGL(wino_dw_kernel<2>, dim3(nb), dim3(256), 0, st, slab, ks, Cout, Cin, Kp, dw);
  return pm_check_launch("wino_dw");
}

int pm_wino_fused_f4(const float* V, const float* U, int Cout, int Kp, const pm_wino_geom& g, float* y, long ypitch, const float* bias, const float* scale,
                     const float* shift, const float* residual, long res_pitch, int relu, hipStream_t st) {
  static pm_lds_optin optin;
  (void)optin(reinterpret_cast<const void*>(&wino_fused_f4_kernel), (int)WF_LDS);
  WinoFusedArgs a;
  a.V = V, a.U = U, a.y = y, a.yp = ypitch, a.Cout = Cout, a.Kp = Kp, a.g = g;
  a.bias = bias, a.scale = scale, a.shift = shift, a.residual = residual, a.rp = res_pitch, a.relu = relu;
  a.ncb = (Cout + WF_CB - 1) / WF_CB;
  const long ntb = (g.tiles + WF_TB - 1) / WF_TB;
  hipLaunchKernelGGL(wino_fused_f4_kernel, dim3((unsigned)(ntb * a.ncb)), dim3(WF_THREADS), WF_LDS, st, a);
  return pm_check_launch("wino_fused_f4");
}
```

### pinthememory_amd/hip/kernels.py

```python
import ctypes
from ctypes import byref

import os
import weakref

import torch

from . import lib as L
from .lib import PmConvEpilogue, PmConvParams, check, ptr, stream, tdesc, workspace


def _lib():
    return L.load()


CONV_PREC = 0
ACT_DTYPE = torch.float32


def set_conv_precision(name):
    global CONV_PREC, ACT_DTYPE
    CONV_PREC = {'f32': 0, 'fp32': 0, 'bf16': 2, 'bf16_operands': 2, 'bf16_staged': 1}[name]
    ACT_DTYPE = torch.bfloat16 if name == 'bf16' else torch.float32

# ... 128 lines not shown
            self.nbytes += nbu
        else:
            del self[key]
        self[key] = ent
        ent.used = True
        version = owner._version
        valid = ent.version == version
        if not valid:
            ent.version = -1
        p.wxf, p.wxf_bytes, p.wxf_valid = ent.buf.data_ptr(), nbu, 1 if valid else 0
        raw, cur = self._stream()
        if valid and ent.event is not None and ent.stream != raw:
            cur.wait_event(ent.event)
        return None if valid else (ent, version)

    def commit(self, *pending):
        raw, cur = self._stream()
        event = cur.record_event()
        for ent, version in pending:
            ent.version, ent.event, ent.stream = version, event, raw

    def forget_events(self):
        for ent in self.values():
            ent.event = ent.stream = None


_U_CACHE = _FilterCache()
clear_filters, forget_filter_events = _U_CACHE.clear, _U_CACHE.forget_events

_REFRESH = {2: ('pm_conv_wxf_refresh_bf16', False), 0: ('pm_conv_wxf_refresh_f32', True)}


def refresh_filters():
    if KEEP_WINOGRAD_U is False or not _U_CACHE or CONV_PREC not in _REFRESH:
        return 0
    entry_point, forward_3x3_only = _REFRESH[CONV_PREC]
    dev = torch.cuda.current_device()
    todo = []
    for ent in _U_CACHE.values():
        if ent.prec != CONV_PREC or ent.device != dev or not ent.used:
            continue
        cout, kh, kw, cin = ent.shape
        if forward_3x3_only and (ent.dgrad or kh != 3 or kw != 3):
            continue
        ent.used = False
        owner = ent.owner()
        if owner is None or owner.data_ptr() != ent.ptr or ent.version == owner._version or not ent.buf.is_cuda:
            continue
        todo.append((ent, owner._version))
    if not todo:
        return 0
    jobs = (L.PmWxfJob * len(todo))()
    for j, (ent, version) in zip(jobs, todo):
        cout, kh, kw, cin = ent.shape
        j.w, j.wxf, j.wxf_bytes, j.cout, j.kh, j.kw, j.cin, j.dgrad = ent.ptr, ent.buf.data_ptr(), ent.nbytes, cout, kh, kw, cin, 1 if ent.dgrad else 0
        ent.version = -1
    check(getattr(_lib(), entry_point)(jobs, len(todo), stream()), entry_point)
    _U_CACHE.commit(*todo)
    return len(todo)


_SIZES = {}
_GEN = [0]


def _sizes(key, fn):
    v = _SIZES.get(key)
    if v is None:
        if len(_SIZES) > 8192:
            _SIZES.clear()
        v = _SIZES[key] = fn()
    return v


_XFORM_COUNT = [0, False]


def filter_transform_count(enable=None):
    if enable is not None:
        _XFORM_COUNT[1] = bool(enable)
    return _XFORM_COUNT[0]


def conv_fwd(x, w_krsc, stride, pad, dil, bias=None, scale=None, shift=None, residual=None, relu=False, out=None, keep_v=None, bn_partials=None, out_dtype=None):
    cout, kh, kw, cin = w_krsc.shape
    n, h, w_, c = x.shape
    assert c == cin, 'conv: Cin mismatch %d vs %d' % (c, cin)
    ho, wo = conv_out_hw(h, w_, kh, stride, pad, dil)
    y = out if out is not None else new((n, ho, wo, cout), x, pitch_pad=True, dtype=out_dtype if out_dtype is not None else ACT_DTYPE)
    assert residual is None or residual.dtype == y.dtype, 'conv_fwd: the fused residual has the dtype of the output'
    xd, yd = tdesc(x), tdesc(y)
    p = L.conv_params(kh, kw, stride, pad, dil, CONV_PREC)
    lib = _lib()
    nbv, nbu, nb, npb = _sizes(('f', x.shape, x.stride(), x.dtype, xd.flags, w_krsc.shape, y.stride(), y.dtype, stride, pad, dil, CONV_PREC, _GEN[0]),
                               lambda: (lib.pm_conv_winograd_v_bytes(byref(xd), byref(yd), byref(p)), lib.pm_conv_wxf_bytes(byref(xd), byref(yd), byref(p)),
                                        lib.pm_conv_workspace(byref(xd), byref(yd), byref(p), 0), lib.pm_conv_bn_partials_bytes(byref(xd), byref(yd), byref(p))))
    if keep_v is not None:
        nbv = nbv if KEEP_WINOGRAD_V else 0
        v = torch.empty(nbv // 4, dtype=torch.float32, device=x.device) if nbv else None
        keep_v.append(v)
        if v is not None:
            p.wino_v, p.wino_v_bytes = v.data_ptr(), nbv
    u_ent = None
    if (kh == 3 and CONV_PREC == 0) or CONV_PREC == 2:
        u_ent = _U_CACHE.lookup(p, w_krsc, nbu)
    if _XFORM_COUNT[1] and p.wxf_valid == 0 and nbu:
        _XFORM_COUNT[0] += 1
    ws = workspace(nb, x.device) if nb else None
    part = None
    if bn_partials is not None:
        ep16 = BN_EPILOGUE16 or (BN_EP16_MIN_BYTES > 0 and y.numel() * 2 >= BN_EP16_MIN_BYTES)
        ep32 = BN_EPILOGUE or (BN_EP_MIN_BYTES > 0 and y.numel() * 4 >= BN_EP_MIN_BYTES)
        npb = npb if ((ep16 if y.dtype == torch.bfloat16 else ep32) and residual is None and not relu and scale is None) else 0
        part = torch.empty(npb // 4, dtype=torch.float32, device=x.device) if npb else None
        bn_partials.append(part)
    ep = None
    if bias is not None or scale is not None or residual is not None or relu or part is not None:
        rd = tdesc(residual) if residual is not None else None
        ep = L.conv_epilogue(ptr(bias), ptr(scale), ptr(shift), rd.ptr if rd else None, rd.pitch if rd else 0, 1 if relu else 0, ptr(part),
                            part.numel() * 4 if part is not None else 0)
    check(lib.pm_conv_fwd(byref(xd), w_krsc.data_ptr(), byref(yd), byref(p), byref(ep) if ep else None, ptr(ws), nb, stream()), 'pm_conv_fwd')
    if u_ent is not None:
        _U_CACHE.commit(u_ent)
    return y


def conv_bwd_data(dy, w_krsc, x_shape, stride, pad, dil, add=None, dtype=None, add_mask=None):
    cout, kh, kw, cin = w_krsc.shape
    dx = new(x_shape, dy, dtype=dtype)
    dyd, dxd = tdesc(dy), tdesc(dx)
    p = L.conv_params(kh, kw, stride, pad, dil, CONV_PREC)
    lib = _lib()
    nb, nbu = _sizes(('d', dy.shape, dy.stride(), dy.dtype, dyd.flags, w_krsc.shape, dx.shape, dx.stride(), dx.dtype, stride, pad, dil, CONV_PREC, _GEN[0]),
                     lambda: (lib.pm_conv_workspace(byref(dxd), byref(dyd), byref(p), 1), lib.pm_conv_wxf_bytes_dgrad(byref(dyd), byref(dxd), byref(p))))
    ws = workspace(nb, dy.device) if nb else None
    ad = tdesc(add) if add is not None else None
    u_ent = _U_CACHE.lookup(p, w_krsc, nbu, dgrad=True) if CONV_PREC == 2 else None
    if add_mask is not None:
        check(lib.pm_conv_bwd_data_masked(byref(dyd), w_krsc.data_ptr(), byref(dxd), byref(p), byref(ad), add_mask.data_ptr(), ptr(ws), nb, stream()), 'pm_conv_bwd_data_masked')
    else:
        check(lib.pm_conv_bwd_data(byref(dyd), w_krsc.data_ptr(), byref(dxd), byref(p), byref(ad) if ad else None, ptr(ws), nb, stream()), 'pm_conv_bwd_data')
    if u_ent is not None:
        _U_CACHE.commit(u_ent)
    return dx


def conv_bwd_weight(x, dy, w_shape_krsc, stride, pad, dil, want_bias=False, wino_v=None, on_stream=None):
    cout, kh, kw, cin = w_shape_krsc
    dw = torch.empty(w_shape_krsc, dtype=torch.float32, device=x.device)
    db = torch.empty(cout, dtype=torch.float32, device=x.device) if want_bias else None
    xd, dyd = tdesc(x), tdesc(dy)
    p = L.conv_params(kh, kw, stride, pad, dil, CONV_PREC)
    if wino_v is not None:
        p.wino_v, p.wino_v_bytes = wino_v.data_ptr(), wino_v.numel() * 4
    lib = _lib()
    nb = _sizes(('w', x.shape, x.stride(), x.dtype, dy.shape, dy.stride(), dy.dtype, w_shape_krsc, stride, pad, dil, CONV_PREC, wino_v is not None, _GEN[0]),
                lambda: lib.pm_conv_workspace(byref(xd), byref(dyd), byref(p), 2))
    raw = stream() if on_stream is None else on_stream.cuda_stream
    ws = workspace(nb, x.device, on_stream)
    check(lib.pm_conv_bwd_weight(byref(xd), byref(dyd), dw.data_ptr(), ptr(db), byref(p), ptr(ws), nb, raw), 'pm_conv_bwd_weight')
    return dw, db


def bn_stats(x):
    c = x.shape[3]
    mom = torch.empty(3 * c, dtype=torch.float32, device=x.device)
    xd = tdesc(x)
    lib = _lib()
    nb = _sizes(('bn', x.shape, x.dtype), lambda: lib.pm_bn_workspace(byref(xd)))
    ws = workspace(nb, x.device)
    check(lib.pm_bn_stats(byref(xd), mom.data_ptr(), ptr(ws), nb, stream()), 'pm_bn_stats')
    return mom


def bn_stats_finalize(x, eps, running_mean=None, running_var=None, momentum=0.1):
    c = x.shape[3]
    mean = torch.empty(c, dtype=torch.float32, device=x.device)
    invstd = torch.empty_like(mean)
    xd = tdesc(x)
    lib = _lib()
    nb = _sizes(('bn', x.shape, x.dtype), lambda: lib.pm_bn_workspace(byref(xd)))
    ws = workspace(nb, x.device)
    check(lib.pm_bn_stats_finalize(byref(xd), eps, mean.data_ptr(), invstd.data_ptr(), ptr(running_mean), ptr(running_var), momentum, ptr(ws), nb, stream()),
          'pm_bn_stats_finalize')
    return mean, invstd


def bn_partials_finalize(part, pixels, c, eps, running_mean=None, running_var=None, momentum=0.1):
    mean = torch.empty(c, dtype=torch.float32, device=part.device)
    invstd = torch.empty_like(mean)
    check(_lib().pm_bn_partials_finalize(part.data_ptr(), pixels, c, eps, mean.data_ptr(), invstd.data_ptr(), ptr(running_mean), ptr(running_var), momentum, None,
                                         stream()), 'pm_bn_partials_finalize')
    return mean, invstd


def bn_partials_moments(part, pixels, c):
    mom = torch.empty(3 * c, dtype=torch.float32, device=part.device)
    check(_lib().pm_bn_partials_finalize(part.data_ptr(), pixels, c, 0.0, None, None, None, None, 0.0, mom.data_ptr(), stream()), 'pm_bn_partials_finalize')
    return mom


def bn_merge(parts, world, c):
    out = torch.empty(3 * c, dtype=torch.float32, device=parts.device)
    check(_lib().pm_bn_merge(parts.data_ptr(), world, c, out.data_ptr(), stream()), 'pm_bn_merge')
    return out


def bn_merge_finalize(parts, world, c, eps, running_mean=None, running_var=None, momentum=0.1):
    mean = torch.empty(c, dtype=torch.float32, device=parts.device)
    invstd = torch.empty_like(mean)
    check(_lib().pm_bn_merge_finalize(parts.data_ptr(), world, c, eps, mean.data_ptr(), invstd.data_ptr(), ptr(running_mean), ptr(running_var), momentum,
                                      stream()), 'pm_bn_merge_finalize')
    return mean, invstd


def bn_finalize(moments, c, eps, running_mean=None, running_var=None, momentum=0.1):
    mean = torch.empty(c, dtype=torch.float32, device=moments.device)
    invstd = torch.empty_like(mean)
    check(_lib().pm_bn_finalize(moments.data_ptr(), c, eps, mean.data_ptr(), invstd.data_ptr(), ptr(running_mean), ptr(running_var), momentum, stream()),
          'pm_bn_finalize')
    return mean, invstd


def bn_fold_multi(table, cs, offs, n, max_c, total, eps):
    arena = torch.empty(2 * total, dtype=torch.float32, device=table.device)
    check(_lib().pm_bn_fold_multi(table.data_ptr(), cs.data_ptr(), offs.data_ptr(), n, max_c, total, eps, arena.data_ptr(), stream()), 'pm_bn_fold_multi')
    return arena


def bn_fold(gamma, beta, running_mean, running_var, eps, conv_bias=None):
    c = gamma.numel()
    scale = torch.empty(c, dtype=torch.float32, device=gamma.device)
    shift = torch.empty_like(scale)
    check(_lib().pm_bn_fold(gamma.data_ptr(), beta.data_ptr(), running_mean.data_ptr(), running_var.data_ptr(), ptr(conv_bias), c, eps, scale.data_ptr(),
                            shift.data_ptr(), stream()), 'pm_bn_fold')
    return scale, shift


def bn_apply(x, mean, invstd, gamma, beta, residual=None, relu=False, out=None, want_mask=False):
    y = out if out is not None else torch.empty_like(x, memory_format=torch.contiguous_format)
    rd = tdesc(residual) if residual is not None else None
    grp = 8 if x.dtype == torch.bfloat16 else 4
    mask = torch.empty((x.shape[0] * x.shape[1] * x.shape[2], x.shape[3] // grp), dtype=torch.uint8, device=x.device) if want_mask else None
# ... 1068 lines not shown
```

### pinthememory_amd/hip/lib.py

```python
import ctypes
import os
from ctypes import POINTER, byref, c_char_p, c_float, c_int, c_int32, c_int64, c_size_t, c_void_p

import torch

_HERE = os.path.dirname(os.path.dirname(os.path.abspath(__file__)))
LIB_PATH = os.environ.get('PM_LIB') or os.path.join(_HERE, 'libpinmem_hip.so')


class PmTensor(ctypes.Structure):
    _fields_ = [('ptr', c_void_p), ('n', c_int32), ('h', c_int32), ('w', c_int32), ('c', c_int32), ('pitch', c_int64), ('dtype', c_int32), ('flags', c_int32)]


PM_F32, PM_BF16 = 0, 1
PM_TF_ZERO_PAD64 = 1


class PmSgdEntry(ctypes.Structure):
    _fields_ = [('param', c_void_p), ('grad', c_void_p), ('momentum_buffer', c_void_p), ('numel', c_int64)]


class PmWxfJob(ctypes.Structure):
    _fields_ = [('w', c_void_p), ('wxf', c_void_p), ('wxf_bytes', c_int64), ('cout', c_int32), ('kh', c_int32), ('kw', c_int32), ('cin', c_int32),
                ('dgrad', c_int32), ('reserved', c_int32)]


class PmConvParams(ctypes.Structure):
    _fields_ = [('struct_size', c_int32), ('kh', c_int32), ('kw', c_int32), ('stride', c_int32), ('pad', c_int32), ('dil', c_int32), ('prec', c_int32),
                ('wino_v', c_void_p), ('wino_v_bytes', c_int64),
                ('wxf', c_void_p), ('wxf_bytes', c_int64), ('wxf_valid', c_int32)]


class PmRouting(ctypes.Structure):
    _fields_ = [('struct_size', c_int32), ('winograd', c_int32), ('winograd_fused', c_int32), ('conv16', c_int32), ('conv16_wide', c_int32),
                ('conv16_persistent', c_int32), ('wgrad16', c_int32), ('bf16_wgrad', c_int32), ('split', c_int32)]


class PmAugImage(ctypes.Structure):
    _fields_ = [('order', ctypes.c_uint8 * 4), ('enabled', ctypes.c_uint8), ('flip', ctypes.c_uint8), ('hue_shift', ctypes.c_uint8), ('reserved', ctypes.c_uint8),
                ('brightness', c_float), ('contrast', c_float), ('saturation', c_float), ('radius', c_int32), ('w', ctypes.c_double * 6)]


class PmGeoImage(ctypes.Structure):
    _fields_ = [('h_in', c_int32), ('w_in', c_int32), ('h', c_int32), ('w', c_int32), ('pad_h', c_int32), ('pad_w', c_int32), ('y1', c_int32), ('x1', c_int32)]


LABEL_SLOTS, LABEL_MAX_COLORS = 256, 128
LABEL_IDS, LABEL_COLORS = 0, 1


class PmLabelTable(ctypes.Structure):
    _fields_ = [('mode', c_int32), ('fill', c_int32), ('lut', ctypes.c_uint8 * 256), ('keys', ctypes.c_uint32 * LABEL_SLOTS), ('vals', ctypes.c_uint8 * LABEL_SLOTS)]


RESAMPLE_MAX_TAPS = 24
RESAMPLE_REC = RESAMPLE_MAX_TAPS + 2
FILTER_BILINEAR, FILTER_BICUBIC = 2, 3


class PmConvEpilogue(ctypes.Structure):
    _fields_ = [('struct_size', c_int64), ('bias', c_void_p), ('scale', c_void_p), ('shift', c_void_p), ('residual', c_void_p),
                ('residual_pitch', c_int64), ('relu', c_int32), ('bn_partials', c_void_p), ('bn_partials_bytes', c_int64)]


def conv_params(kh, kw, stride, pad, dil, prec=0):
    return PmConvParams(ctypes.sizeof(PmConvParams), kh, kw, stride, pad, dil, prec)


def conv_epilogue(*fields):
    return PmConvEpilogue(ctypes.sizeof(PmConvEpilogue), *fields)


ABI_VERSION = 460


class PinmemError(RuntimeError):
    pass


_T, _P, _E = POINTER(PmTensor), POINTER(PmConvParams), POINTER(PmConvEpilogue)
_vp, _sz, _i, _f, _i64 = c_void_p, c_size_t, c_int, c_float, c_int64

SIGNATURES = {
    'pm_last_error': (c_char_p, []),
    'pm_version': (c_int, []),
    'pm_conv_winograd_v_bytes': (_sz, [_T, _T, _P]),
    'pm_conv_wxf_bytes': (_sz, [_T, _T, _P]),
    'pm_conv_wxf_bytes_dgrad': (_sz, [_T, _T, _P]),
    'pm_conv_wxf_refresh_bf16': (_i, [_vp, _i, _vp]),
    'pm_conv_wxf_refresh_f32': (_i, [_vp, _i, _vp]),
    'pm_conv_workspace': (_sz, [_T, _T, _P, _i]),
    'pm_conv_fwd': (_i, [_T, _vp, _T, _P, _E, _vp, _sz, _vp]),
    'pm_conv_bwd_data': (_i, [_T, _vp, _T, _P, _T, _vp, _sz, _vp]),
    'pm_conv_bwd_data_masked': (_i, [_T, _vp, _T, _P, _T, _vp, _vp, _sz, _vp]),
    'pm_conv_bwd_weight': (_i, [_T, _T, _vp, _vp, _P, _vp, _sz, _vp]),
    'pm_set_winograd': (_i, [_i]),
    'pm_set_winograd_fused': (_i, [_i]),
    'pm_set_conv16': (_i, [_i]),
    'pm_profile_enable': (_i, [_i]),
    'pm_profile_dump': (_i, [ctypes.c_char_p]),
    'pm_profile_read': (_i, [_i, _i, _i, _i, _i, POINTER(ctypes.c_double), POINTER(ctypes.c_double), POINTER(c_int64), _i]),
    'pm_profile_read_prec': (_i, [_i, _i, _i, _i, _i, _i, POINTER(ctypes.c_double), POINTER(ctypes.c_double), POINTER(c_int64), _i]),
    'pm_profile_read_bytes': (_i, [_i, _i, _i, _i, _i, _i, POINTER(ctypes.c_double)]),
    'pm_bn_workspace': (_sz, [_T]),
    'pm_bn_stats': (_i, [_T, _vp, _vp, _sz, _vp]),
    'pm_bn_merge': (_i, [_vp, _i, _i, _vp, _vp]),
    'pm_bn_merge_finalize': (_i, [_vp, _i, _i, _f, _vp, _vp, _vp, _vp, _f, _vp]),
    'pm_bn_finalize': (_i, [_vp, _i, _f, _vp, _vp, _vp, _vp, _f, _vp]),
    'pm_bn_stats_finalize': (_i, [_T, _f, _vp, _vp, _vp, _vp, _f, _vp, _sz, _vp]),
    'pm_bn_fold': (_i, [_vp, _vp, _vp, _vp, _vp, _i, _f, _vp, _vp, _vp]),
    'pm_bn_fold_multi': (_i, [_vp, _vp, _vp, _i, _i, _i, _f, _vp, _vp]),
    'pm_bn_apply': (_i, [_T, _vp, _vp, _vp, _vp, _T, _i, _T, _vp]),
    'pm_bn_apply_mask': (_i, [_T, _vp, _vp, _vp, _vp, _T, _i, _T, _vp, _vp]),
    'pm_bn_bwd_reduce_mask': (_i, [_T, _vp, _T, _vp, _vp, _T, _vp, _vp, _sz, _vp]),
    'pm_bn_apply_mask_affine': (_i, [_T, _vp, _vp, _vp, _vp, _T, _vp, _vp, _vp, _vp, _i, _T, _vp, _vp]),
    'pm_bn_bwd_apply_mask': (_i, [_T, _vp, _T, _vp, _vp, _vp, _vp, _f, _T, _vp]),
    'pm_bn_bwd_reduce': (_i, [_T, _T, _T, _vp, _vp, _vp, _vp, _i, _T, _vp, _vp, _sz, _vp]),
    'pm_bn_bwd_apply': (_i, [_T, _T, _T, _vp, _vp, _vp, _vp, _vp, _f, _i, _T, _T, _vp]),
    'pm_relu_bwd': (_i, [_T, _T, _T, _vp]),
    'pm_add': (_i, [_T, _T, _T, _vp]),
    'pm_add_n': (_i, [POINTER(_T), _i, _T, _vp]),
    'pm_copy': (_i, [_T, _T, _vp]),
    'pm_scale_shift_act': (_i, [_T, _vp, _vp, _T, _i, _T, _vp]),
    'pm_maxpool3x3s2_fwd': (_i, [_T, _T, _vp, _vp]),
    'pm_maxpool3x3s2_bwd': (_i, [_T, _vp, _T, _vp]),
    'pm_maxpool3x3s2_bn_relu_fwd': (_i, [_T, _vp, _vp, _vp, _vp, _T, _vp, _vp]),
    'pm_bn_bwd_reduce_pool': (_i, [_T, _vp, _T, _vp, _vp, _vp, _vp, _vp, _vp, _sz, _vp]),
    'pm_bn_bwd_apply_pool': (_i, [_T, _vp, _T, _vp, _vp, _vp, _vp, _vp, _f, _T, _vp]),
    'pm_global_avgpool_fwd': (_i, [_T, _T, _vp]),
    'pm_global_avgpool_bwd': (_i, [_T, _T, _i, _vp]),
    'pm_resize_bilinear_fwd': (_i, [_T, _T, _vp]),
    'pm_resize_bilinear_bwd': (_i, [_T, _T, _i, _vp]),
    'pm_resize_bilinear_bwd_workspace': (_sz, [_T, _T]),
    'pm_resize_bilinear_bwd_separable': (_i, [_T, _T, _i, _vp, _sz, _vp]),
    'pm_resize_bilinear_hp_fwd': (_i, [_T, _T, _i, _vp]),
    'pm_softmax_mean_update': (_i, [_T, _vp, _i, _vp]),
    'pm_sliding_stitch': (_i, [_T, _vp, _i, _i, _i, _i, _vp, _i, _vp]),
    'pm_argmax_f64': (_i, [_vp, _i, _i, _i, _i, _vp, _vp, _vp]),
    'pm_sliding_eval_workspace': (_sz, [_i, _i, _i, _i]),
    'pm_sliding_eval': (_i, [_vp, _i, _i, _i, _i, _i64, _i, _vp, _i, _i, _i, _i, _i, _vp, _vp, _i, _vp, _vp, _vp, _i, _vp, _sz, _vp]),
    'pm_sliding_eval_finish': (_i, [_vp, _i, _i, _i, _i, _vp, _vp, _i, _vp, _vp, _vp, _sz, _vp]),
    'pm_image_u8_to_nhwc4': (_i, [_vp, _i64, POINTER(c_float), POINTER(c_float), _vp, _vp]),
    'pm_labels_u8_to_i64': (_i, [_vp, _i64, _vp, _vp]),
    'pm_aug_blur_weights': (_i, [ctypes.c_double, POINTER(c_int32), POINTER(ctypes.c_double)]),
    'pm_augment_workspace': (_sz, [_i]),
    'pm_augment_u8': (_i, [_vp, _i, _i, _i, _vp, c_int32, POINTER(c_float), POINTER(c_float), _vp, _vp, _vp, _sz, _vp]),
    'pm_labels_u8_flip_to_i64': (_i, [_vp, _i, _i, _i, _vp, c_int32, _vp, _vp]),
    'pm_resample_tables': (_i, [_vp, c_int32, _i, _i, _i, _i, _vp, _vp, _vp, _vp]),
    'pm_resample_crop_u8': (_i, [_vp, _vp, _i, _i, _i, _vp, c_int32, _vp, _vp, _vp, _vp, _i, _i, _i, _vp, _vp, _vp]),
    'pm_resize_axis_tables': (_i, [_i, _i, _i, _vp]),
    'pm_eval_tiles_u8': (_i, [_vp, _i, _i, _vp, _vp, _i, _i, _vp, _i, _i, _i, _i, POINTER(c_float), POINTER(c_float), _vp, _vp]),
    'pm_label_table_ids': (_i, [_vp, _vp, _i, _vp, c_int32]),
    'pm_label_table_colors': (_i, [_vp, _vp, _i, _i, _vp, c_int32]),
    'pm_labels_decode_u8': (_i, [_vp, _i, _i, _i, _i, _vp, _i, c_int32, _vp, _vp, _vp]),
    'pm_resample_crop_decode_u8': (_i, [_vp, _vp, _i, _i, _i, _vp, c_int32, _vp, _vp, _vp, _vp, _i, _i, _i, _i, _vp, _i, c_int32, _vp, _vp, _vp, _vp]),
    'pm_nchw_to_nhwc': (_i, [_vp, _i, _T, _vp]),
    'pm_nhwc_to_nchw': (_i, [_T, _vp, _vp]),
    'pm_label_nearest': (_i, [_vp, _i, _i, _i, _vp, _i, _i, _vp]),
    'pm_upsample_ce_workspace': (_sz, [_i, _i, _i]),
    'pm_upsample_ce_fwd': (_i, [_T, _f, _vp, _i, _i, _vp, _vp, _sz, _vp]),
    'pm_upsample_ce_bwd_workspace': (_sz, [_T, _i, _i]),
    'pm_upsample_ce_bwd': (_i, [_T, _f, _vp, _i, _i, _vp, _vp, _T, _vp, _sz, _vp]),
    'pm_upsample_ce_field_bytes': (_sz, [_T, _i, _i]),
    'pm_upsample_ce_fwd_field': (_i, [_T, _f, _vp, _i, _i, _vp, _vp, _vp, _sz, _vp]),
    'pm_upsample_ce_bwd_field': (_i, [_T, _f, _i, _i, _vp, _vp, _vp, _T, _vp]),
    'pm_upsample_wce_loss_floats': (_sz, [_i]),
    'pm_upsample_wce_workspace': (_sz, [_i, _i, _i]),
    'pm_upsample_wce_fwd': (_i, [_T, _f, _vp, _i, _i, _vp, _i64, _i, _vp, _vp, _sz, _vp]),
    'pm_upsample_wce_fwd_field': (_i, [_T, _f, _vp, _i, _i, _vp, _i64, _i, _vp, _vp, _vp, _sz, _vp]),
    'pm_upsample_wce_bwd_field': (_i, [_T, _f, _i, _i, _i, _vp, _vp, _vp, _T, _vp]),
    'pm_label_class_weights_workspace': (_sz, [_i]),
    'pm_label_class_weights': (_i, [_vp, _i, _i, _i, _i, ctypes.c_double, _i, _i, _vp, _vp, _sz, _vp]),
    'pm_relax_border_bits': (_i, [_vp, _i, _i, _i, _i, _i, ctypes.c_uint32, _vp, _vp]),
    'pm_multihot_to_bits': (_i, [_vp, _i, _i, _i, _i, _vp, _vp]),
    'pm_relax_class_weights_workspace': (_sz, [_i]),
    'pm_relax_class_weights': (_i, [_vp, _i, _i, _i, _i, ctypes.c_double, _i, _i, _vp, _vp, _sz, _vp]),
    'pm_upsample_relax_workspace': (_sz, [_i, _i, _i]),
    'pm_upsample_relax_loss_floats': (_sz, [_i]),
# ... 137 lines not shown
```

### pinthememory_amd/hip/ops.py

```python
import os as _os

import torch

from . import kernels as K
from . import lib as L
from .. import dist as D


def nhwc(t):
    v = t.permute(0, 2, 3, 1)
    n, h, w, c = v.shape
    sn, sh, sw, sc = v.stride()
    pitch = sw if w > 1 else (sh if h > 1 else (sn if n > 1 else c))
    ok = (sc == 1 or c == 1) and pitch >= c and (h == 1 or w == 1 or sh == w * pitch) and (n == 1 or h * w == 1 or sn == h * w * pitch)
    if ok and v.dtype == torch.float32:
        return v
    if v.dtype == torch.bfloat16:
        if ok and pitch % 8 == 0 and c % 8 == 0 and v.data_ptr() % 16 == 0:
            return v
        return v.contiguous()
    if h * w == 1:
        return v.contiguous().float()
    return K.nchw_to_nhwc(t.float())

# ... 24 lines not shown


_nbt_pending = []


def flush_bn_counters():
    if _nbt_pending:
        torch._foreach_add_(_nbt_pending, 1)
        _nbt_pending.clear()


_OVERLAP_ENV = _os.environ.get('PM_OVERLAP_WGRAD')
OVERLAP_WGRAD = True if _OVERLAP_ENV is None else _OVERLAP_ENV == '1'


def overlap_wgrad():
    if not OVERLAP_WGRAD:
        return False
    return not (_OVERLAP_ENV is None and K.CONV_PREC == 2 and K.ACT_DTYPE == torch.bfloat16)


_side = {}
_proxy = {}


def masked_stream(n_cus, device=None, first=0):
    import ctypes
    dev = torch.cuda.current_device() if device is None else device
    total = torch.cuda.get_device_properties(dev).multi_processor_count
    n_cus = max(1, min(int(n_cus), total))
    words = (total + 31) // 32
    mask = (ctypes.c_uint32 * words)()
    picked = {(first + (i * total) // n_cus) % total for i in range(n_cus)}
    for cu in picked:
        mask[cu // 32] |= 1 << (cu % 32)
    hip = ctypes.CDLL('libamdhip64.so')
    st = ctypes.c_void_p()
    with torch.cuda.device(dev):
        err = hip.hipExtStreamCreateWithCUMask(ctypes.byref(st), ctypes.c_uint32(words), mask)
    if err != 0 or not st.value:
        raise RuntimeError('hipExtStreamCreateWithCUMask(%d CUs) failed: %d' % (n_cus, err))
    return torch.cuda.ExternalStream(st.value, device=dev)


WGRAD_CUS = int(_os.environ.get('PM_WGRAD_CUS', '0'))


def _side_stream():
    dev = torch.cuda.current_device()
    if dev not in _side:
        _side[dev] = masked_stream(WGRAD_CUS, dev) if WGRAD_CUS > 0 else torch.cuda.Stream(device=dev)
    return _side[dev]


class _Defer(torch.autograd.Function):
    @staticmethod
    def forward(ctx, w):
        return w.view_as(w)

    @staticmethod
    def backward(ctx, g):
        L.stream_obj().wait_stream(_side_stream())
        return g


def begin_forward():
    flush_bn_counters()
    _proxy.clear()


def defer_weights(module):
    if not (overlap_wgrad() and torch.is_grad_enabled()):
        return
    for m in module.modules():
        if isinstance(m, torch.nn.Conv2d) and m.bias is None and m.weight.requires_grad and id(m.weight) not in _proxy:
            _proxy[id(m.weight)] = _Defer.apply(m.weight)


def _w(weight):
    p = _proxy.get(id(weight))
    return (p, True) if p is not None else (weight, False)


def _wgrad(x, dy, wshape, geom, want_bias=False, deferred=False, wino_v=None):
    if not deferred:
        return K.conv_bwd_weight(x, dy, wshape, *geom, want_bias=want_bias, wino_v=wino_v)
    side, main = _side_stream(), L.stream_obj()
    ev = torch.cuda.Event()
    ev.record(main)
    side.wait_event(ev)
    out = K.conv_bwd_weight(x, dy, wshape, *geom, want_bias=want_bias, wino_v=wino_v, on_stream=side)
    if wino_v is not None:
        wino_v.record_stream(side)
    x.record_stream(side)
    dy.record_stream(side)
    for t in out:
        if t is not None:
            t.record_stream(side)
    return out


commit_done = {}


def wait_commit():
    if not commit_done or not torch.cuda.is_available():
        return
    ev = commit_done.pop(torch.cuda.current_device(), None)
    if ev is not None:
        torch.cuda.current_stream().wait_event(ev)


def _same_exchange(groups, widths):
    return D.is_dist() and all(g is not None and g is groups[0] for g in groups) and len(set(widths)) == 1


def _bn_train_stats_multi(ys, bns, partials):
    n = len(ys)
    if n > 1 and not _same_exchange([b.group for b in bns], [y.shape[3] for y in ys]):
        return [_bn_train_stats(y, bn, part) for y, bn, part in zip(ys, bns, partials)]
    pixels = [y.shape[0] * y.shape[1] * y.shape[2] for y in ys]
    if bns[0].group is None:
        y, bn, part = ys[0], bns[0], partials[0]
        if part is not None:
            return [K.bn_partials_finalize(part, pixels[0], y.shape[3], bn.eps, bn.running_mean, bn.running_var, bn.momentum)]
        return [K.bn_stats_finalize(y, bn.eps, bn.running_mean, bn.running_var, bn.momentum)]
    c = ys[0].shape[3]
    moms = [K.bn_partials_moments(part, px, c) if part is not None else K.bn_stats(y) for y, part, px in zip(ys, partials, pixels)]
    flat, world = D.gather_moments(moms[0] if n == 1 else torch.cat(moms), bns[0].group)
    parts = flat.view(world, n, 3 * c)
    return [K.bn_merge_finalize(parts[:, i].contiguous().view(-1), world, c, bn.eps, bn.running_mean, bn.running_var, bn.momentum) for i, bn in enumerate(bns)]


def _bn_train_stats(y, bn, partials=None):
    return _bn_train_stats_multi([y], [bn], [partials])[0]


def _bn_train_fwd(y, gamma, beta, bn, residual, relu, out=None, partials=None):
    mean, invstd = _bn_train_stats(y, bn, partials)
    return K.bn_apply(y, mean, invstd, gamma, beta, residual=residual, relu=relu, out=out), mean, invstd


class _BnSums:

    def __init__(self, n, c, group, device):
        self.c, self.group, self.with_count = c, group, group is not None
        self.len = 2 * c + (1 if self.with_count else 0)
        self.stride = (self.len + 3) // 4 * 4
        self.local = torch.empty((n - 1) * self.stride + self.len, dtype=torch.float32, device=device)
        self.summed = self.local

    def slot(self, i):
        return self.local[i * self.stride:i * self.stride + self.len]

    def exchange(self):
        if self.group is not None:
            self.summed = D.all_reduce_sum_copy(self.local, self.group)

    def total(self, i):
        return self.summed[i * self.stride:i * self.stride + self.len]

    def count(self, y):
        return -1.0 if self.with_count else float(y.shape[0] * y.shape[1] * y.shape[2])

    def grads(self, i):
        s = self.slot(i)
        return s[self.c:2 * self.c], s[:self.c]


def _bn_train_bwd(dv, o, y, mean, invstd, gamma, beta, relu, group, want_dres, has_res, mask=None):
    mode = 0 if not relu else (1 if has_res else 2)
    hand_over = mode == 1 and want_dres
    S = _BnSums(1, y.shape[3], group, y.device)
    if hand_over and mask is not None:
        _, gm = K.bn_bwd_reduce_mask(dv, mask, y, mean, invstd, want_gmask=True, with_count=S.with_count, sums=S.slot(0))
    else:
        _, gm = K.bn_bwd_reduce(dv, o, y, mean, invstd, mode, gamma, beta, want_gmask=hand_over, with_count=S.with_count, sums=S.slot(0))
    S.exchange()
    if hand_over:
        dy, dres = K.bn_bwd_apply(gm, None, y, mean, invstd, gamma, S.total(0), S.count(y), 0, False)[0], gm
    else:
        dy, dres = K.bn_bwd_apply(dv, o, y, mean, invstd, gamma, S.total(0), S.count(y), mode, want_dres, beta)
    return (dy, dres, *S.grads(0))


def _bn_bwd_masked(dv, mask, y, mean, invstd, gamma, group):
    S = _BnSums(1, y.shape[3], group, y.device)
    K.bn_bwd_reduce_mask(dv, mask, y, mean, invstd, want_gmask=False, with_count=S.with_count, sums=S.slot(0))
    S.exchange()
    return (K.bn_bwd_apply_mask(dv, mask, y, mean, invstd, gamma, S.total(0), S.count(y)), *S.grads(0))


class _Bottleneck(torch.autograd.Function):

    @staticmethod
    def forward(ctx, x, w1, g1, b1, w2, g2, b2, w3, g3, b3, wd, gd, bd, geoms, bns, deferred):
        xv = nhwc(x)
        k1, k2, k3 = K.krsc(w1), K.krsc(w2), K.krsc(w3)
        ps = []
        y1 = K.conv_fwd(xv, k1, *geoms[0], bn_partials=ps)
        o1, m1, i1 = _bn_train_fwd(y1, g1, b1, bns[0], None, True, partials=ps[0])
        kv = []
        y2 = K.conv_fwd(o1, k2, *geoms[1], keep_v=kv, bn_partials=ps)
        o2, m2, i2 = _bn_train_fwd(y2, g2, b2, bns[1], None, True, partials=ps[1])
        y3 = K.conv_fwd(o2, k3, *geoms[2], bn_partials=ps)
        m3 = None
        if wd is not None:
            kd = K.krsc(wd)
            yd = K.conv_fwd(xv, kd, *geoms[3], bn_partials=ps)
            fold = y3.dtype == torch.float32 and yd.dtype == torch.float32
            if fold or _same_exchange([bns[3].group, bns[2].group], [yd.shape[3], y3.shape[3]]):
                (md, idd), (m3, i3) = _bn_train_stats_multi([yd, y3], [bns[3], bns[2]], [ps[3], ps[2]])
                res = None if fold else K.bn_apply(yd, md, idd, gd, bd, residual=None, relu=False)
            else:
                res, md, idd = _bn_train_fwd(yd, gd, bd, bns[3], None, False, partials=ps[3])
        else:
            kd = yd = md = idd = None
            res = xv
        if m3 is None:
            m3, i3 = _bn_train_stats(y3, bns[2], ps[2])
        if res is None:
            out, mask3 = K.bn_apply_res_affine(y3, m3, i3, g3, b3, yd, md, idd, gd, bd, relu=True, want_mask=True)
        else:
            out, mask3 = K.bn_apply(y3, m3, i3, g3, b3, residual=res, relu=True, want_mask=True)
        ctx.geoms, ctx.groups, ctx.has_ds, ctx.deferred = geoms, [b.group for b in bns], wd is not None, deferred
        ctx.save_for_backward(xv, k1, k2, k3, kd, y1, o1, y2, o2, y3, yd, out, m1, i1, m2, i2, m3, i3, md, idd, g1, g2, g3, gd, b1, b2, b3, kv[0], mask3)
        return nchw(out)

    @staticmethod
    def backward(ctx, dout):
        xv, k1, k2, k3, kd, y1, o1, y2, o2, y3, yd, out, m1, i1, m2, i2, m3, i3, md, idd, g1, g2, g3, gd, b1, b2, b3, v2, mask3 = ctx.saved_tensors
        ge, gr, df = ctx.geoms, ctx.groups, ctx.deferred
        dv = _grad_view(dout)
        pair = None
        if ctx.has_ds and _same_exchange([gr[2], gr[3]], [y3.shape[3], yd.shape[3]]):
            S = _BnSums(2, y3.shape[3], gr[2], y3.device)
            _, gm = K.bn_bwd_reduce_mask(dv, mask3, y3, m3, i3, want_gmask=True, with_count=True, sums=S.slot(0))
            K.bn_bwd_reduce(gm, None, yd, md, idd, 0, gd, None, want_gmask=False, with_count=True, sums=S.slot(1))
            S.exchange()
            dy3, _ = K.bn_bwd_apply(gm, None, y3, m3, i3, g3, S.total(0), -1.0, 0, False)
            dyd, _ = K.bn_bwd_apply(gm, None, yd, md, idd, gd, S.total(1), -1.0, 0, False, None)
            dres, (dg3, db3), pair = gm, S.grads(0), (dyd, *S.grads(1))
        elif dv.dtype == torch.float32 and K.CONV_PREC != 2:
            dy3, dg3, db3 = _bn_bwd_masked(dv, mask3, y3, m3, i3, g3, gr[2])
            dres = None
        else:
            dy3, dres, dg3, db3 = _bn_train_bwd(dv, out, y3, m3, i3, g3, b3, True, gr[2], True, True, mask=mask3)
        dw3, _ = _wgrad(o2, dy3, tuple(k3.shape), ge[2], deferred=df[2])
        do2 = K.conv_bwd_data(dy3, k3, tuple(o2.shape), *ge[2])
        dy2, _, dg2, db2 = _bn_train_bwd(do2, o2, y2, m2, i2, g2, b2, True, gr[1], False, False)
        dw2, _ = _wgrad(o1, dy2, tuple(k2.shape), ge[1], deferred=df[1], wino_v=v2)
        do1 = K.conv_bwd_data(dy2, k2, tuple(o1.shape), *ge[1])
        dy1, _, dg1, db1 = _bn_train_bwd(do1, o1, y1, m1, i1, g1, b1, True, gr[0], False, False)
        dw1, _ = _wgrad(xv, dy1, tuple(k1.shape), ge[0], deferred=df[0])
        dwd = dgd = dbd = None
        skip, skip_mask = (dres, None) if dres is not None else (dv, mask3)
        if ctx.has_ds:
            if pair is not None:
                dyd, dgd, dbd = pair
            elif dres is None:
                dyd, dgd, dbd = _bn_bwd_masked(dv, mask3, yd, md, idd, gd, gr[3])
            else:
                dyd, _, dgd, dbd = _bn_train_bwd(dres, None, yd, md, idd, gd, None, False, gr[3], False, False)
            dwdk, _ = _wgrad(xv, dyd, tuple(kd.shape), ge[3], deferred=df[3])
            dwd = dwdk.permute(0, 3, 1, 2)
            skip, skip_mask = (K.conv_bwd_data(dyd, kd, tuple(xv.shape), *ge[3]) if ctx.needs_input_grad[0] else None), None
        dx = nchw(K.conv_bwd_data(dy1, k1, tuple(xv.shape), *ge[0], add=skip, add_mask=skip_mask)) if ctx.needs_input_grad[0] else None
        p = lambda d: d.permute(0, 3, 1, 2)
        return dx, p(dw1), dg1, db1, p(dw2), dg2, db2, p(dw3), dg3, db3, dwd, dgd, dbd, None, None, None


FOLD_BATCH = _os.environ.get('PM_FOLD_BATCH', '1') == '1'
_fold_cache = None
fold_misses = 0
last_prefold_event = None


class prefold:
    def __init__(self, model):
        self.model, self.active = model, False

    def __enter__(self):
        global _fold_cache, last_prefold_event
        last_prefold_event = None
        m = self.model
        if not FOLD_BATCH or m.training or torch.is_grad_enabled() or _fold_cache is not None:
            return self
        bns = getattr(m, '_pm_bn_list', None)
        if bns is None:
            bns = [b for b in m.modules() if isinstance(b, torch.nn.modules.batchnorm._BatchNorm)]
            m.__dict__['_pm_bn_list'] = bns
        bns = [b for b in bns if b.running_mean is not None and b.weight is not None and b.running_mean.is_cuda and not b.training]
        if not bns or len({b.eps for b in bns}) != 1:
            return self
        ptrs = tuple(t.data_ptr() for b in bns for t in (b.weight, b.bias, b.running_mean, b.running_var))
        plan = m.__dict__.get('_pm_fold_plan')
        if plan is None or plan[0] != ptrs:
            dev = bns[0].running_mean.device
            cs = [b.num_features for b in bns]
            offs, tot = [], 0
            for c in cs:
                offs.append(tot)
                tot += (c + 3) // 4 * 4
            as_i64 = [p - (1 << 64) if p >= (1 << 63) else p for p in ptrs]
            plan = (ptrs, torch.tensor(as_i64, dtype=torch.int64, device=dev), torch.tensor(cs, dtype=torch.int32, device=dev),
                    torch.tensor(offs, dtype=torch.int32, device=dev), cs, offs, tot)
            m.__dict__['_pm_fold_plan'] = plan
        _, table, dcs, doffs, cs, offs, tot = plan
        arena = K.bn_fold_multi(table, dcs, doffs, len(cs), max(cs), tot, bns[0].eps)
        _fold_cache = {b.running_mean.data_ptr(): (arena[o:o + c], arena[tot + o:tot + o + c]) for b, c, o in zip(bns, cs, offs)}
        self.active = True
        last_prefold_event = torch.cuda.current_stream().record_event() if len(bns) == len(m.__dict__['_pm_bn_list']) else None
        return self

    def __exit__(self, *exc):
        global _fold_cache
        if self.active:
            _fold_cache = None
        return False


class _ConvBnAct(torch.autograd.Function):

    @staticmethod
    def forward(ctx, x, w, bias, gamma, beta, residual, geom, bn, relu, out, deferred=False):
        stride, pad, dil = geom
        xv, wk = nhwc(x), K.krsc(w)
        rv = nhwc(residual) if residual is not None else None
        ov = nhwc(out) if out is not None else None
        ctx.geom, ctx.relu, ctx.train, ctx.deferred = geom, relu, bn.training, deferred and bias is None
        needs_grad = bn.grad_enabled and any(ctx.needs_input_grad[:6])
        if not bn.training and not needs_grad:
            hit = _fold_cache.get(bn.running_mean.data_ptr()) if (_fold_cache is not None and bias is None) else None
            if hit is None:
                global fold_misses
                fold_misses += 1
            scale, shift = hit if hit is not None else K.bn_fold(gamma, beta, bn.running_mean, bn.running_var, bn.eps, bias)
            o = K.conv_fwd(xv, wk, stride, pad, dil, scale=scale, shift=shift, residual=rv, relu=relu, out=ov)
            return nchw(o)
        kv, ps = [], []
        y = K.conv_fwd(xv, wk, stride, pad, dil, bias=bias, keep_v=kv if ctx.needs_input_grad[1] else None, bn_partials=ps if bn.training else None)
        if bn.training:
            o, mean, invstd = _bn_train_fwd(y, gamma, beta, bn, rv, relu, ov, partials=ps[0])
        else:
            mean, invstd = bn.running_mean, torch.rsqrt(bn.running_var + bn.eps)
            o = K.bn_apply(y, mean, invstd, gamma, beta, residual=rv, relu=relu, out=ov)
        ctx.group, ctx.has_bias, ctx.has_res = bn.group, bias is not None, residual is not None
        ctx.save_for_backward(xv, wk, y, o, mean, invstd, gamma, beta, kv[0] if kv else None)
        return nchw(o)

    @staticmethod
    def backward(ctx, dout):
        xv, wk, y, o, mean, invstd, gamma, beta, vk = ctx.saved_tensors
        stride, pad, dil = ctx.geom
        dv = _grad_view(dout)
        want_dres = ctx.has_res and ctx.needs_input_grad[5]
        if ctx.train:
            dy, dres, dgamma, dbeta = _bn_train_bwd(dv, o, y, mean, invstd, gamma, beta, ctx.relu, ctx.group, want_dres, ctx.has_res)
        else:
            c = y.shape[3]
            mode = 0 if not ctx.relu else (1 if ctx.has_res else 2)
            sums, g = K.bn_bwd_reduce(dv, o, y, mean, invstd, mode, gamma, beta, want_gmask=mode != 0)
            g = dv if g is None else g
            dy = K.scale_shift_act(g, gamma * invstd, torch.zeros_like(gamma))
            dres, dgamma, dbeta = (g if want_dres else None), sums[c:], sums[:c]
        dx = nchw(K.conv_bwd_data(dy, wk, tuple(xv.shape), stride, pad, dil, dtype=xv.dtype)) if ctx.needs_input_grad[0] else None
        dw = db = None
        if ctx.needs_input_grad[1] or (ctx.has_bias and ctx.needs_input_grad[2]):
            dwk, db = _wgrad(xv, dy, tuple(wk.shape), (stride, pad, dil), want_bias=ctx.has_bias, deferred=ctx.deferred, wino_v=vk)
            dw = dwk.permute(0, 3, 1, 2)
        return dx, dw, db, dgamma, dbeta, (nchw(dres) if dres is not None else None), None, None, None, None, None


class _Stem(torch.autograd.Function):

    @staticmethod
    def forward(ctx, x, w, gamma, beta, geom, bn):
        xv, wk = nhwc(x), K.krsc(w)
        kv, ps = [], []
        y = K.conv_fwd(xv, wk, *geom, keep_v=kv if ctx.needs_input_grad[1] else None, bn_partials=ps)
        mean, invstd = _bn_train_stats(y, bn, ps[0])
        out, arg = K.maxpool_bn_relu_fwd(y, mean, invstd, gamma, beta)
        ctx.geom, ctx.group = geom, bn.group
        ctx.save_for_backward(xv, wk, y, mean, invstd, gamma, beta, arg, kv[0] if kv else None)
        return nchw(out)

    @staticmethod
    def backward(ctx, dout):
        xv, wk, y, mean, invstd, gamma, beta, arg, vk = ctx.saved_tensors
        dv = _grad_view(dout)
        S = _BnSums(1, y.shape[3], ctx.group, y.device)
        K.bn_bwd_reduce_pool(dv, arg, y, mean, invstd, gamma, beta, with_count=S.with_count, sums=S.slot(0))
        S.exchange()
        dy = K.bn_bwd_apply_pool(dv, arg, y, mean, invstd, gamma, beta, S.total(0), S.count(y))
        dx = nchw(K.conv_bwd_data(dy, wk, tuple(xv.shape), *ctx.geom, dtype=xv.dtype)) if ctx.needs_input_grad[0] else None
        dw = None
        if ctx.needs_input_grad[1]:
            dwk, _ = _wgrad(xv, dy, tuple(wk.shape), ctx.geom, wino_v=vk)
            dw = dwk.permute(0, 3, 1, 2)
        return (dx, dw, *S.grads(0), None, None)


def stem_tail(x, w, conv, bn):
    st = BNState(bn)
    if st.training and torch.is_grad_enabled() and K.ACT_DTYPE == torch.float32 and x.dtype == torch.float32 and w.shape[0] % 4 == 0:
        return _Stem.apply(x, w, bn.weight, bn.bias, _geom(conv), st)
    return maxpool3x3s2(_ConvBnAct.apply(x, w, None, bn.weight, bn.bias, None, _geom(conv), st, True, None))


class _ConvBnActN(torch.autograd.Function):

    @staticmethod
    def forward(ctx, n, geoms, bns, outs, deferreds, *ts):
        xs, ws, gammas, betas = ts[0:n], ts[n:2 * n], ts[2 * n:3 * n], ts[3 * n:4 * n]
        xvs, wks = [nhwc(x) for x in xs], [K.krsc(w) for w in ws]
        ys, kvs, parts = [], [], []
        for i in range(n):
            kv, ps = [], []
            ys.append(K.conv_fwd(xvs[i], wks[i], *geoms[i], keep_v=kv if ctx.needs_input_grad[5 + n + i] else None, bn_partials=ps))
            kvs.append(kv[0] if kv else None)
            parts.append(ps[0])
        stats = _bn_train_stats_multi(ys, bns, parts)
        os_ = [K.bn_apply(ys[i], stats[i][0], stats[i][1], gammas[i], betas[i], residual=None, relu=True, out=nhwc(outs[i]) if outs[i] is not None else None) for i in range(n)]
        ctx.n, ctx.geoms, ctx.group, ctx.deferreds = n, geoms, bns[0].group, deferreds
        ctx.save_for_backward(*xvs, *wks, *ys, *os_, *[st[0] for st in stats], *[st[1] for st in stats], *gammas, *betas, *kvs)
        return tuple(nchw(o) for o in os_)

    @staticmethod
    def backward(ctx, *douts):
        n = ctx.n
        sv = ctx.saved_tensors
        xvs, wks, ys, os_, means, invs, gammas, betas, kvs = (sv[i * n:(i + 1) * n] for i in range(9))
        S = _BnSums(n, ys[0].shape[3], ctx.group, ys[0].device)
        for i in range(n):
            K.bn_bwd_reduce(_grad_view(douts[i]), os_[i], ys[i], means[i], invs[i], 2, gammas[i], betas[i], want_gmask=False, with_count=True, sums=S.slot(i))
        S.exchange()
        dxs, dws, dgs, dbs = [], [], [], []
        for i in range(n):
            dy, _ = K.bn_bwd_apply(_grad_view(douts[i]), os_[i], ys[i], means[i], invs[i], gammas[i], S.total(i), -1.0, 2, False, betas[i])
            dxs.append(nchw(K.conv_bwd_data(dy, wks[i], tuple(xvs[i].shape), *ctx.geoms[i], dtype=xvs[i].dtype)) if ctx.needs_input_grad[5 + i] else None)
            dwk, _ = _wgrad(xvs[i], dy, tuple(wks[i].shape), ctx.geoms[i], deferred=ctx.deferreds[i], wino_v=kvs[i])
            dws.append(dwk.permute(0, 3, 1, 2))
            dg, db = S.grads(i)
            dgs.append(dg), dbs.append(db)
        return (None, None, None, None, None, *dxs, *dws, *dgs, *dbs)


def conv_bn_act_n(xs, seqs, outs):
    convs, bns_m = [q[0] for q in seqs], [q[1] for q in seqs]
    ok = (torch.is_grad_enabled() and all(b.training for b in bns_m) and all(cv.bias is None for cv in convs)
          and _same_exchange([D.bn_group(b) for b in bns_m], [cv.out_channels for cv in convs]))
    if not ok:
        return [conv_bn_act(x, cv, bn, relu=True, out=o) for x, cv, bn, o in zip(xs, convs, bns_m, outs)]
    states = [BNState(b) for b in bns_m]
# ... 145 lines not shown


class _MemRead(torch.autograd.Function):

    @staticmethod
    def forward(ctx, x, mem, noise, noise_q=None, with_pq=False):
        xv = nhwc(x)
        mem = mem.contiguous()
        if with_pq:
            qr, score, pmem, pq = K.mem_read_fwd_pq(xv, mem, noise, noise_q)
        else:
            qr, score, pmem = K.mem_read_fwd(xv, mem, noise)
        n, h, w, _ = xv.shape
        m = mem.shape[0]
        ctx.save_for_backward(xv, mem, pmem)
        score, pmem = score.view(n, h, w, m), pmem.view(n, h, w, m)
        ctx.with_pq = with_pq
        if with_pq:
            pq = pq.view(n, h, w, m)
            ctx.mark_non_differentiable(pmem, pq)
            return nchw(qr), score, pmem, pq
        ctx.mark_non_differentiable(pmem)
        return nchw(qr), score, pmem

    @staticmethod
    def backward(ctx, dqr, dscore, _dp, _dq=None):
        xv, mem, pmem = ctx.saved_tensors
        n, h, w, d = xv.shape
        dq = _grad_view(dqr) if dqr is not None else torch.zeros((n, h, w, 2 * d), dtype=torch.float32, device=xv.device)
        ds = dscore.contiguous() if dscore is not None else None
        dx, dmem = K.mem_read_bwd(xv, mem, pmem, dq, ds, want_dmem=ctx.needs_input_grad[1])
        return nchw(dx), dmem, None, None, None


class _MemWriteAccum(torch.autograd.Function):

    @staticmethod
    def forward(ctx, z, labels, m):
        zv = nhwc(z)
        labels = labels.contiguous()
        ctx.m = m
        ctx.save_for_backward(zv, labels)
        return K.mem_write_accum(zv, labels, m, normalize=True)

    @staticmethod
    def backward(ctx, dnomden):
        zv, labels = ctx.saved_tensors
        m, d = ctx.m, zv.shape[3]
        dnom = dnomden[:(m + 1) * d].contiguous()
        return nchw(K.mem_write_accum_bwd(zv, labels, m, dnom, normalize=True)), None, None


class _MemWriteUpdate(torch.autograd.Function):

    @staticmethod
    def forward(ctx, mem, nomden, momentum):
        mem = mem.contiguous()
        out, u = K.mem_write_update(mem, nomden, momentum, want_u=True)
        ctx.momentum = momentum
        ctx.save_for_backward(u, nomden)
        return out

    @staticmethod
    def backward(ctx, dout):
        u, nomden = ctx.saved_tensors
        m, d = u.shape
        dnom = K.mem_write_update_bwd(u, nomden, ctx.momentum, dout.contiguous())
        g = torch.zeros_like(nomden)
        g[:(m + 1) * d] = dnom.reshape(-1)
        return None, g, None


def _geom(conv):
    assert conv.kernel_size[0] == conv.kernel_size[1] and conv.stride[0] == conv.stride[1] and conv.groups == 1
    assert conv.padding[0] == conv.padding[1] and conv.dilation[0] == conv.dilation[1]
    return conv.stride[0], conv.padding[0], conv.dilation[0]


def conv_bn_act(x, conv, bn, relu=True, residual=None, out=None):
    w, deferred = _w(conv.weight)
    return _ConvBnAct.apply(x, w, conv.bias, bn.weight, bn.bias, residual, _geom(conv), BNState(bn), relu, out, deferred)


def bottleneck(x, blk):
    ds = blk.downsample
    mods = [(blk.conv1, blk.bn1), (blk.conv2, blk.bn2), (blk.conv3, blk.bn3)] + ([(ds[0], ds[1])] if ds is not None else [])
    geoms = [_geom(c) for c, _ in mods]
    bns = [BNState(b) for _, b in mods]
    ws = [_w(c.weight) for c, _ in mods]
    wd, gd, bd = (ws[3][0], ds[1].weight, ds[1].bias) if ds is not None else (None, None, None)
    return _Bottleneck.apply(x, ws[0][0], blk.bn1.weight, blk.bn1.bias, ws[1][0], blk.bn2.weight, blk.bn2.bias,
                             ws[2][0], blk.bn3.weight, blk.bn3.bias, wd, gd, bd, geoms, bns, [d for _, d in ws] + [False])


def conv(x, conv_mod):
    return _Conv.apply(x, conv_mod.weight, conv_mod.bias, _geom(conv_mod))


def conv_raw(x, weight, bias, geom):
    return _Conv.apply(x, weight, bias, geom)


def instance_norm_act(x, weight, bias, eps=1e-5, relu=True):
    assert (weight is None) == (bias is None), 'instance_norm_act: weight and bias come together'
    return _InstNormAct.apply(x, weight, bias, float(eps), bool(relu))


def instance_norm_module(x, m, relu=True):
    assert isinstance(m, torch.nn.InstanceNorm2d) and not m.track_running_stats, 'instance norm with running statistics is not served'
    return instance_norm_act(x, m.weight, m.bias, m.eps, relu)


def maxpool3x3s2(x):
    return _MaxPool.apply(x)


def global_avgpool(x):
    return _GlobalAvgPool.apply(x)


def resize(x, size, out=None):
    return _Resize.apply(x, size, out)


def concat_buffer(like, channels, hw):
    return nchw(K.new((like.shape[0], hw[0], hw[1], sum(channels)), like, dtype=like.dtype if like.dtype == torch.bfloat16 else torch.float32))


def concat(buf, parts):
    return _Concat.apply(buf, *parts)


def add(a, b):
    return _Add.apply(a, b)


class _Cast(torch.autograd.Function):

    @staticmethod
    def forward(ctx, x, dtype):
        ctx.src = x.dtype
        return nchw(K.cast(nhwc(x), dtype))

    @staticmethod
    def backward(ctx, g):
        return nchw(K.cast(_grad_view(g), ctx.src)), None


def cast(x, dtype):
    return x if x.dtype == dtype else _Cast.apply(x, dtype)


def upsample_ce(logits, labels, inv_temp=1.0):
    if not K.upsample_ce_fused_ok(nhwc(logits), tuple(labels.shape[1:])):
        full = resize(logits, tuple(labels.shape[1:]))
        return torch.nn.functional.cross_entropy(full * float(inv_temp), labels, ignore_index=255, reduction='mean')
    return _UpsampleLoss.apply(logits, labels, float(inv_temp), bool(torch.is_grad_enabled() and logits.requires_grad))


def weighted_ce(full, labels, weights, per_image):
    lp = torch.nn.functional.log_softmax(full, dim=1)
    weights = weights.to(device=full.device, dtype=lp.dtype)
    if weights.dim() == 1 and not per_image:
        return torch.nn.functional.nll_loss(lp, labels, weight=weights, ignore_index=255, reduction='mean')
    rows = weights.expand(full.shape[0], -1) if weights.dim() == 1 else weights
    num = [torch.nn.functional.nll_loss(lp[b:b + 1], labels[b:b + 1], weight=rows[b], ignore_index=255, reduction='sum') for b in range(full.shape[0])]
# ... 58 lines not shown
```

### pinthememory_amd/network/deepv3plus.py

```python
import torch
import torch.nn as nn

from . import Resnet, memory
from .mynn import Norm2d, Upsample, channels_last_weights, initialize_weights
from ..hip import kernels as K
from ..hip import ops
from .. import loss as _loss


def _cbr(cin, cout, k, **kw):
    return nn.Sequential(nn.Conv2d(cin, cout, kernel_size=k, bias=False, **kw), Norm2d(cout), nn.ReLU(inplace=True))


def run_cbr(seq, x, out=None, residual=None):
    return ops.conv_bn_act(x, seq[0], seq[1], relu=True, out=out, residual=residual)


def fused_ce_ok(criterion):
    return (isinstance(criterion, nn.CrossEntropyLoss) and criterion.ignore_index == 255 and criterion.reduction == 'mean'
            and criterion.weight is None and getattr(criterion, 'label_smoothing', 0.0) == 0.0)


def _plain_nll(c):
    return c.ignore_index == 255 and getattr(c, 'reduction', 'mean') == 'mean' and getattr(c, 'label_smoothing', 0.0) == 0.0 and getattr(c, 'size_average', True) in (None, True)
# ... 112 lines not shown
            return_loss = [loss1, self._aux_loss(aux_out, gts, aux_gts)]
            if self.args.memory:
                return_loss += [mem_output, writeloss, readloss]
            return_loss.append(inter_feature)
            return return_loss
        outputs = [dec2 if self.eval_logits_lowres else Upsample(dec2, x_size[2:])]
        if self.args.memory:
            outputs.append(mem_output)
        outputs.append(inter_feature)
        return outputs

    def _run_memory(self, dec0_up, gts, memory_writing, writing_detach):
        if gts is not None and gts.dim() == 4:
            raise ValueError('the memory needs class indices, not a multi-hot relaxed-border target (the reference fails here too): pass int64 labels as gts, '
                             'the relaxed criterion builds the border sets from them')
        dec0_up, sq, sm, readloss, writeloss = self.memory(dec0_up, gts, memory_writing, writing_detach)
        return dec0_up, [sq, sm, dec0_up.detach()], readloss, writeloss


class DeepV3Plus(_Base):
    def __init__(self, num_classes, trunk='resnet-101', criterion=None, criterion_aux=None, variant='D', skip='m1', skip_num=48, args=None):
        super().__init__()
        self.criterion, self.criterion_aux, self.variant, self.args, self.trunk = criterion, criterion_aux, variant, args, trunk
        Resnet.check_wt_layer(args.wt_layer)
        assert not args.use_wtloss, 'whitening is out of scope of the pinmem hot path'
        if trunk != 'resnet-50':
            raise ValueError("Not a valid network arch")
        self._adopt_trunk(trunk)

        def dilate(layer, d):
            for n, m in layer.named_modules():
                if 'conv2' in n:
                    m.dilation, m.padding, m.stride = (d, d), (d, d), (1, 1)
                elif 'downsample.0' in n:
                    m.stride = (1, 1)
        if variant == 'D':
            dilate(self.layer3, 2), dilate(self.layer4, 4)
            os = 8
        elif variant == 'D16':
            dilate(self.layer4, 2)
            os = 16
        else:
            raise ValueError('unknown deepv3 variant: {}'.format(variant))
        self.output_stride = os
        self.aspp = _AtrousSpatialPyramidPoolingModule(2048, 256, output_stride=os)
        self.bot_fine = _cbr(256, 48, 1)
        self.bot_aspp = _cbr(1280, 256, 1)
        self.final1 = nn.Sequential(*(list(_cbr(304, 256, 3, padding=1)) + list(_cbr(256, 256, 3, padding=1))))
        self.final2 = nn.Sequential(nn.Conv2d(256, num_classes, kernel_size=1, bias=True))
        self.dsn = nn.Sequential(nn.Conv2d(1024, 512, kernel_size=3, stride=1, padding=1), Norm2d(512), nn.ReLU(inplace=True), nn.Dropout2d(0.1),
                                 nn.Conv2d(512, num_classes, kernel_size=1, stride=1, padding=0, bias=True))
        initialize_weights(self.dsn)
        initialize_weights(self.aspp)
        initialize_weights(self.bot_aspp)
        initialize_weights(self.bot_fine)
        initialize_weights(self.final1)
        initialize_weights(self.final2)
        self.eps = 1e-5
        self.whitening = False
        self.three_input_layer = False
        self.cov_matrix_layer, self.cov_type = [], []
        self._make_memory()
        channels_last_weights(self)

    def forward(self, x, gts=None, aux_gts=None, img_gt=None, visualize=False, cal_covstat=False, apply_wtloss=True,
                memory_writing=False, writing_detach=True):
        with ops.prefold(self):
            return self._forward(x, gts, aux_gts, img_gt, visualize, cal_covstat, apply_wtloss, memory_writing, writing_detach)

    def _forward(self, x, gts, aux_gts, img_gt, visualize, cal_covstat, apply_wtloss, memory_writing, writing_detach):
        assert not cal_covstat and not visualize, 'whitening statistics are out of scope'
        x_size = x.size()
        low_level, aux_out, x = self._trunk(x)
        x = self.aspp(x)
        dec0_up = run_cbr(self.bot_aspp, x)
        inter_feature = dec0_up
        mem_output = writeloss = readloss = None
        if self.args.memory:
            dec0_up, mem_output, readloss, writeloss = self._run_memory(dec0_up, gts, memory_writing, writing_detach)
        buf = ops.concat_buffer(low_level, [48, 256], low_level.shape[2:])
        dec0_fine = run_cbr(self.bot_fine, low_level, out=buf[:, :48])
        dec0_up = ops.resize(dec0_up, low_level.size()[2:], out=buf[:, 48:])
        dec0 = ops.concat(buf, [dec0_fine, dec0_up])
        dec1 = ops.conv_bn_act(dec0, self.final1[0], self.final1[1], relu=True)
        dec1 = ops.conv_bn_act(dec1, self.final1[3], self.final1[4], relu=True)
        dec2 = ops.conv(dec1, self.final2[0])
        return self._finish(dec2, x_size, aux_out, gts, aux_gts, mem_output, writeloss, readloss, inter_feature)


def DeepR50V3PlusD_OS8(args, num_classes, criterion, criterion_aux):
    print("Model : DeepLabv3+, Backbone : ResNet-50")
    return DeepV3Plus(num_classes, trunk='resnet-50', criterion=criterion, criterion_aux=criterion_aux, variant='D', skip='m1', args=args)


def DeepR50V3PlusD(args, num_classes, criterion, criterion_aux):
    print("Model : DeepLabv3+, Backbone : ResNet-50")
    return DeepV3Plus(num_classes, trunk='resnet-50', criterion=criterion, criterion_aux=criterion_aux, variant='D16', skip='m1', args=args)
```

Baseline: 159.9.

## Fuse BatchNorm+ReLU into Winograd input transforms for forward and backward passes

Adds Winograd input-transform variants that apply the preceding BatchNorm affine and ReLU while loading. The normalized activation no longer has to be materialized before a 3x3 conv in bottlenecks and the decoder pair. In backward, a fused BN-backward transform writes the dgrad V and the wgrad Z directly, so a separate dy tensor and the dy transform are skipped. This adds new entry points, a new autograd function for the decoder conv pair, and stream/event plumbing for the deferred wgrad. The BN affine is recomputed in several transforms, and the path only applies when all three conv routes are Winograd.

```diff
diff --git a/include/pinmem_hip.h b/include/pinmem_hip.h
--- a/include/pinmem_hip.h
+++ b/include/pinmem_hip.h
@@ -71,6 +71,16 @@
                             const pm_tensor* add, const uint8_t* add_mask, void* ws, size_t ws_bytes, void* stream);
 int pm_conv_bwd_weight(const pm_tensor* x, const pm_tensor* dy, float* dw_krsc, float* dbias, const pm_conv_params* p,
                        void* ws, size_t ws_bytes, void* stream);
+size_t pm_conv_winograd_z_bytes(const pm_tensor* x, const pm_tensor* y, const pm_conv_params* p);
+int pm_conv_fwd_bn(const float* x, int64_t x_pitch, int n, int h, int w, int cin, const float* mean, const float* invstd, const float* gamma, const float* beta,
+                   const float* w_krsc, float* y, int64_t y_pitch, int cout, const pm_conv_params* p, const pm_conv_epilogue* ep, void* ws, size_t ws_bytes,
+                   void* stream);
+int pm_conv_bwd_data_bn(const float* g, int64_t g_pitch, const float* y, int64_t y_pitch, int n, int h, int w, int cout, const float* mean, const float* invstd,
+                        const float* gamma, const float* beta, const float* sums, float count, const float* w_krsc, float* dx, int64_t dx_pitch, int cin,
+                        const pm_conv_params* p, const float* add, int64_t add_pitch, void* z, size_t z_bytes, float* dy, int64_t dy_pitch, void* z_event, void* ws,
+                        size_t ws_bytes, void* stream);
+int pm_conv_bwd_weight_z(const float* x, int64_t x_pitch, int n, int h, int w, int cin, int cout, const void* z, size_t z_bytes, float* dw_krsc,
+                         const pm_conv_params* p, void* ws, size_t ws_bytes, void* stream);
 
 typedef struct pm_routing {
   int32_t struct_size;
diff --git a/pinthememory_amd/csrc/conv_igemm.hip b/pinthememory_amd/csrc/conv_igemm.hip
--- a/pinthememory_amd/csrc/conv_igemm.hip
+++ b/pinthememory_amd/csrc/conv_igemm.hip
@@ -507,12 +507,16 @@
 inline size_t wino_ws(const WinoPlan& wp) { return wp.v_bytes + wp.m_bytes + wp.u_bytes; }
 
 int wino_conv(const pm_tensor* xin, const float* w, int w_cout, int w_cin, bool dgrad, const pm_tensor* yout, const WinoPlan& wp,
-              const pm_conv_epilogue& ep, void* ws, hipStream_t st, float* v_keep = nullptr, float* u_ext = nullptr, bool u_valid = false) {
+              const pm_conv_epilogue& ep, void* ws, hipStream_t st, float* v_keep = nullptr, float* u_ext = nullptr, bool u_valid = false,
+              const pm_wino_bn* in_bn = nullptr, bool v_ready = false) {
   float* V = v_keep ? v_keep : (float*)ws;
   float* Mo = (float*)((char*)ws + wp.v_bytes);
   float* U = u_ext ? u_ext : (float*)((char*)ws + wp.v_bytes + wp.m_bytes);
   const int cout = yout->c;
-  if (int e = pm_wino_input_xf((const float*)xin->ptr, xin->pitch, xin->c, wp.Kp, wp.g, V, st)) return e;
+  if (!v_ready)
+    if (int e = in_bn ? pm_wino_input_bn_xf((const float*)xin->ptr, xin->pitch, xin->c, wp.Kp, wp.g, *in_bn, V, st)
+                      : pm_wino_input_xf((const float*)xin->ptr, xin->pitch, xin->c, wp.Kp, wp.g, V, st))
+      return e;
   if (!(u_ext && u_valid))
     if (int e = pm_wino_filter_xf(w, w_cout, w_cin, wp.Kp, dgrad, wp.g.m, U, st)) return e;
   const pm_tensor xv = {V, 1, 1, (int32_t)wp.g.tiles, wp.Kp, wp.Kp};
@@ -556,14 +560,15 @@
 inline size_t wino_wgrad_ws(const WinoPlan& wp, const WinoWgradPlan& q) { return wp.v_bytes + wp.m_bytes + q.slab_bytes; }
 
 int wino_wgrad(const pm_tensor* x, const pm_tensor* dy, float* dw, const WinoPlan& wp, const WinoWgradPlan& q, void* ws, hipStream_t st,
-               float* v_kept = nullptr) {
+               float* v_kept = nullptr, float* z_pre = nullptr) {
   float* V = v_kept ? v_kept : (float*)ws;
-  float* Z = (float*)((char*)ws + wp.v_bytes);
+  float* Z = z_pre ? z_pre : (float*)((char*)ws + wp.v_bytes);
   float* slab = (float*)((char*)ws + wp.v_bytes + wp.m_bytes);
   const int cout = dy->c;
   if (!v_kept)
     if (int e = pm_wino_input_xf((const float*)x->ptr, x->pitch, x->c, wp.Kp, wp.g, V, st)) return e;
-  if (int e = pm_wino_dy_xf((const float*)dy->ptr, dy->pitch, cout, wp.g, Z, st)) return e;
+  if (!z_pre)
+    if (int e = pm_wino_dy_xf((const float*)dy->ptr, dy->pitch, cout, wp.g, Z, st)) return e;
   const pm_tensor xv = {V, 1, 1, (int32_t)wp.g.tiles, wp.Kp, wp.Kp};
   const pm_tensor zv = {Z, 1, 1, (int32_t)wp.g.tiles, cout, cout};
   const pm_conv_params p1 = {(int32_t)sizeof(pm_conv_params), 1, 1, 1, 0, 1, 0};
@@ -1137,6 +1142,19 @@
   const pm_conv_params tp = tier_params(p0, dy, dx);
   return route_conv(MODE_DGRAD, dx, dy, &tp).wxf_bytes;
 }
+static size_t wino_z_bytes(const pm_tensor* x, const pm_tensor* y, const pm_conv_params* p) {
+  if (!pm_is_f32(x) || !pm_is_f32(y)) return 0;
+  const ConvRoute rf = route_conv(MODE_FWD, x, y, p), rd = route_conv(MODE_DGRAD, x, y, p), rw = route_conv(MODE_WGRAD, x, y, p);
+  if (rf.kind != R_WINO || rd.kind != R_WINO || rw.kind != R_WINO_WGRAD || rf.v_keep_bytes == 0) return 0;
+  const pm_wino_geom &a = rf.wino.g, &b = rd.wino.g, &c = rw.wino.g;
+  if (a.m != c.m || b.m != c.m || a.tiles != c.tiles || b.tiles != c.tiles) return 0;
+  return rw.wino.m_bytes;
+}
+extern "C" size_t pm_conv_winograd_z_bytes(const pm_tensor* x, const pm_tensor* y, const pm_conv_params* p0) {
+  if (!x || !y || !p0 || check_common(x, y, p0) != PM_OK) return 0;
+  const pm_conv_params tp = tier_params(p0, x, y);
+  return wino_z_bytes(x, y, &tp);
+}
 extern "C" size_t pm_conv_bn_partials_bytes(const pm_tensor* x, const pm_tensor* y, const pm_conv_params* p0) {
   if (!x || !y || !p0 || check_common(x, y, p0) != PM_OK) return 0;
   const pm_conv_params tp = tier_params(p0, x, y);
@@ -1162,8 +1180,17 @@
   return pm_wino_filter_xf_multi(w.data(), U.data(), cout.data(), cin.data(), kp.data(), m.data(), n, (hipStream_t)stream);
 }
 
-extern "C" int pm_conv_fwd(const pm_tensor* x, const float* w, const pm_tensor* y, const pm_conv_params* p0,
-                           const pm_conv_epilogue* ep, void* ws, size_t ws_bytes, void* stream) {
+static int check_wino_bn(const char* who, const pm_wino_bn& bn, bool backward) {
+  PM_REQUIRE(bn.mean && bn.invstd && bn.gamma && bn.beta && (!backward || bn.sums), PM_EINVAL, "%s: null BatchNorm constants", who);
+  PM_REQUIRE(pm_aligned16(bn.mean) && pm_aligned16(bn.invstd) && pm_aligned16(bn.gamma) && pm_aligned16(bn.beta) && pm_aligned16(bn.sums), PM_EINVAL,
+             "%s: BatchNorm constants must be 16-byte aligned", who);
+  return PM_OK;
+}
+
+inline pm_tensor f32_view(const void* ptr, int n, int h, int w, int c, int64_t pitch) { return pm_tensor{const_cast<void*>(ptr), n, h, w, c, pitch, PM_F32, 0}; }
+
+static int conv_fwd_entry(const pm_tensor* x, const pm_wino_bn* in_bn, const float* w, const pm_tensor* y, const pm_conv_params* p0, const pm_conv_epilogue* ep, void* ws,
+                   size_t ws_bytes, void* stream) {
   if (int e = check_common(x, y, p0)) return e;
   const pm_conv_params tp = tier_params(p0, x, y);
   const pm_conv_params* p = &tp;
@@ -1181,11 +1208,13 @@
   }
   PM_REQUIRE(ws_bytes >= r.ws_bytes && (ws || r.ws_bytes == 0), PM_EWORKSPACE, "conv_fwd: workspace %zu < %zu", ws_bytes, r.ws_bytes);
   hipStream_t st = (hipStream_t)stream;
+  PM_REQUIRE(!in_bn || r.kind == R_WINO, PM_EUNSUPPORTED, "conv_fwd_bn: the input BatchNorm is evaluated by the Winograd input transform only (this call routes to %s)",
+             r.kind == R_BF16 ? "the bf16 kernels" : "the implicit-GEMM kernels");
   switch (r.kind) {
     case R_WINO: {
       float* keep = (p->wino_v && (size_t)p->wino_v_bytes >= r.wino.v_bytes) ? (float*)p->wino_v : nullptr;
       float* uext = (p->wxf && (size_t)p->wxf_bytes >= r.wino.u_bytes) ? (float*)p->wxf : nullptr;
-      return wino_conv(x, w, y->c, x->c, false, y, r.wino, e0, ws, st, keep, uext, p->wxf_valid != 0);
+      return wino_conv(x, w, y->c, x->c, false, y, r.wino, e0, ws, st, keep, uext, p->wxf_valid != 0, in_bn);
     }
     case R_BF16: {
       char* wext = (p->wxf && (size_t)p->wxf_bytes >= r.b16.wb_bytes) ? (char*)p->wxf : nullptr;
@@ -1195,6 +1224,20 @@
       PM_REQUIRE(pm_is_f32(x), PM_EUNSUPPORTED, "conv_fwd: a bf16 input needs at least 32 channels (got %d)", x->c);
       return conv_direct<MODE_FWD>(x, y, w, p, r.pl, e0, ws, st);
   }
+}
+
+extern "C" int pm_conv_fwd(const pm_tensor* x, const float* w, const pm_tensor* y, const pm_conv_params* p0, const pm_conv_epilogue* ep, void* ws, size_t ws_bytes,
+                           void* stream) {
+  return conv_fwd_entry(x, nullptr, w, y, p0, ep, ws, ws_bytes, stream);
+}
+
+extern "C" int pm_conv_fwd_bn(const float* x, int64_t x_pitch, int n, int h, int w_, int cin, const float* mean, const float* invstd, const float* gamma, const float* beta,
+                              const float* w, float* y, int64_t y_pitch, int cout, const pm_conv_params* p0, const pm_conv_epilogue* ep, void* ws, size_t ws_bytes,
+                              void* stream) {
+  const pm_wino_bn bn = {mean, invstd, gamma, beta, nullptr, 0.f, 0};
+  if (int e = check_wino_bn("conv_fwd_bn", bn, false)) return e;
+  const pm_tensor xt = f32_view(x, n, h, w_, cin, x_pitch), yt = f32_view(y, n, h, w_, cout, y_pitch);
+  return conv_fwd_entry(&xt, &bn, w, &yt, p0, ep, ws, ws_bytes, stream);
 }
 
 extern "C" int pm_conv_bwd_data(const pm_tensor* dy, const float* w, const pm_tensor* dx, const pm_conv_params* p0, const pm_tensor* add,
@@ -1234,6 +1277,56 @@
   }
 }
 
+extern "C" int pm_conv_bwd_data_bn(const float* g_ptr, int64_t g_pitch, const float* y_ptr, int64_t y_pitch, int n, int h, int w_, int cout, const float* mean,
+                                   const float* invstd, const float* gamma, const float* beta, const float* sums, float count, const float* w, float* dx_ptr,
+                                   int64_t dx_pitch, int cin, const pm_conv_params* p0, const float* add_ptr, int64_t add_pitch, void* z, size_t z_bytes, float* dy_ptr,
+                                   int64_t dy_pitch, void* z_event, void* ws, size_t ws_bytes, void* stream) {
+  const pm_tensor gt = f32_view(g_ptr, n, h, w_, cout, g_pitch), yt = f32_view(y_ptr, n, h, w_, cout, y_pitch), dxt = f32_view(dx_ptr, n, h, w_, cin, dx_pitch);
+  const pm_tensor addt = f32_view(add_ptr, n, h, w_, cin, add_pitch), dyt = f32_view(dy_ptr, n, h, w_, cout, dy_pitch);
+  const pm_tensor *g = &gt, *y = &yt, *dx = &dxt, *add = add_ptr ? &addt : nullptr, *dy = dy_ptr ? &dyt : nullptr;
+  if (int e = check_common(dx, g, p0)) return e;
+  PM_REQUIRE(y->ptr && pm_vec_ok(y) && y->pitch >= y->c, PM_EINVAL, "conv_bwd_data_bn: y null, or rows not 16-byte aligned");
+  const pm_wino_bn bn = {mean, invstd, gamma, beta, sums, count > 0.f ? 1.f / count : 0.f, count > 0.f ? 0 : 1};
+  if (int e = check_wino_bn("conv_bwd_data_bn", bn, true)) return e;
+  PM_REQUIRE((z != nullptr) != (dy != nullptr), PM_EINVAL, "conv_bwd_data_bn: exactly one of z and dy");
+  PM_REQUIRE(!dy || (pm_vec_ok(dy) && dy->pitch >= dy->c), PM_EINVAL, "conv_bwd_data_bn: dy rows must be 16-byte aligned");
+  PM_REQUIRE(!add || (pm_vec_ok(add) && add->pitch >= add->c), PM_EINVAL, "conv_bwd_data_bn: `add` rows must be 16-byte aligned");
+  PM_REQUIRE(w && pm_aligned16(w), PM_EINVAL, "conv_bwd_data_bn: weight null or unaligned");
+  const pm_conv_params tp = tier_params(p0, g, dx);
+  const ConvRoute r = route_conv(MODE_DGRAD, dx, g, &tp);
+  PM_REQUIRE(r.kind == R_WINO, PM_EUNSUPPORTED, "conv_bwd_data_bn: the BatchNorm input gradient is evaluated by the Winograd transforms only (this data gradient is off that route)");
+  PM_REQUIRE(ws && ws_bytes >= r.ws_bytes, PM_EWORKSPACE, "conv_bwd_data_bn: workspace %zu < %zu", ws_bytes, r.ws_bytes);
+  if (z) {
+    const size_t zb = wino_z_bytes(dx, g, &tp);
+    PM_REQUIRE(zb != 0, PM_EUNSUPPORTED, "conv_bwd_data_bn: the weight gradient of this convolution is off the Winograd route (pm_conv_winograd_z_bytes == 0): pass dy");
+    PM_REQUIRE(z_bytes >= zb && pm_aligned16(z), PM_EINVAL, "conv_bwd_data_bn: z %zu < %zu bytes, or unaligned", z_bytes, zb);
+  }
+  hipStream_t st = (hipStream_t)stream;
+  if (int e = pm_wino_bn_bwd_xf((const float*)g->ptr, g->pitch, (const float*)y->ptr, y->pitch, g->c, r.wino.Kp, r.wino.g, bn, (float*)ws, (float*)z,
+                                dy ? (float*)dy->ptr : nullptr, dy ? dy->pitch : 0, st))
+    return e;
+  if (z_event) PM_REQUIRE(hipEventRecord((hipEvent_t)z_event, st) == hipSuccess, PM_ELAUNCH, "conv_bwd_data_bn: hipEventRecord failed");
+  const pm_conv_epilogue e1 = {(int64_t)sizeof(pm_conv_epilogue), nullptr, nullptr, nullptr, add ? (const float*)add->ptr : nullptr, add ? add->pitch : 0, 0};
+  return wino_conv(g, w, g->c, dx->c, true, dx, r.wino, e1, ws, st, nullptr, nullptr, false, nullptr, true);
+}
+
+extern "C" int pm_conv_bwd_weight_z(const float* x_ptr, int64_t x_pitch, int n, int h, int w_, int cin, int cout, const void* z, size_t z_bytes, float* dw,
+                                    const pm_conv_params* p0, void* ws, size_t ws_bytes, void* stream) {
+  PM_REQUIRE(x_ptr, PM_EINVAL, "conv_bwd_weight_z: x null (with a kept V its values are not read, but its shape and pitch are checked)");
+  const pm_tensor xt = f32_view(x_ptr, n, h, w_, cin, x_pitch), yt = f32_view(z, n, h, w_, cout, cout);
+  const pm_tensor *x = &xt, *y = &yt;
+  if (int e = check_common(x, y, p0)) return e;
+  PM_REQUIRE(dw && pm_aligned16(dw), PM_EINVAL, "conv_bwd_weight_z: dw null or unaligned");
+  const pm_conv_params tp = tier_params(p0, x, y);
+  const size_t zb = wino_z_bytes(x, y, &tp);
+  PM_REQUIRE(zb != 0, PM_EUNSUPPORTED, "conv_bwd_weight_z: this weight gradient is off the Winograd route (pm_conv_winograd_z_bytes == 0)");
+  PM_REQUIRE(z && pm_aligned16(z) && z_bytes >= zb, PM_EINVAL, "conv_bwd_weight_z: z %zu < %zu bytes, null or unaligned", z_bytes, zb);
+  const ConvRoute r = route_conv(MODE_WGRAD, x, y, &tp);
+  PM_REQUIRE(ws && ws_bytes >= r.ws_bytes, PM_EWORKSPACE, "conv_bwd_weight_z: workspace %zu < %zu", ws_bytes, r.ws_bytes);
+  float* vk = (tp.wino_v && (size_t)tp.wino_v_bytes >= r.wino.v_bytes) ? (float*)tp.wino_v : nullptr;
+  return wino_wgrad(x, y, dw, r.wino, r.wino_w, ws, (hipStream_t)stream, vk, (float*)z);
+}
+
 extern "C" int pm_conv_bwd_weight(const pm_tensor* x0, const pm_tensor* dy0, float* dw, float* dbias, const pm_conv_params* p0, void* ws,
                                   size_t ws_bytes, void* stream) {
   if (int e = check_common(x0, dy0, p0)) return e;
diff --git a/pinthememory_amd/csrc/pm_common.h b/pinthememory_amd/csrc/pm_common.h
--- a/pinthememory_amd/csrc/pm_common.h
+++ b/pinthememory_amd/csrc/pm_common.h
@@ -43,7 +43,15 @@
   long tiles;
 };
 pm_wino_geom pm_wino_make_geom(int n, int h, int w, int d, int m);
+struct pm_wino_bn {
+  const float *mean, *invstd, *gamma, *beta, *sums;
+  float host_inv_n;
+  int dev_count;
+};
 int pm_wino_input_xf(const float* x, long pitch, int C, int Kp, const pm_wino_geom& g, float* V, hipStream_t st);
+int pm_wino_input_bn_xf(const float* x, long pitch, int C, int Kp, const pm_wino_geom& g, const pm_wino_bn& bn, float* V, hipStream_t st);
+int pm_wino_bn_bwd_xf(const float* g, long gpitch, const float* y, long ypitch, int C, int Kp, const pm_wino_geom& geo, const pm_wino_bn& bn, float* V, float* Z,
+                      float* dy, long dypitch, hipStream_t st);
 int pm_wino_filter_xf(const float* w, int Cout, int Cin, int Kp, bool dgrad, int m, float* U, hipStream_t st);
 int pm_wino_filter_xf_multi(const float* const* w, float* const* U, const int* cout, const int* cin, const int* kp, const int* m, int n, hipStream_t st);
 int pm_wino_output_xf(const float* M, int Cout, const pm_wino_geom& g, float* y, long ypitch, const float* bias, const float* scale, const float* shift,
diff --git a/pinthememory_amd/csrc/winograd.hip b/pinthememory_amd/csrc/winograd.hip
--- a/pinthememory_amd/csrc/winograd.hip
+++ b/pinthememory_amd/csrc/winograd.hip
@@ -108,8 +108,35 @@
   return t;
 }
 
-template <int MT, int W>
-__global__ __launch_bounds__(256) void wino_input_kernel(const float* __restrict__ x, long xp, int C, int Kp, const pm_wino_geom g, float* __restrict__ V) {
+struct WinoRaw {
+  template <int W>
+  struct K {};
+  template <int W>
+  __device__ __forceinline__ void load(int, K<W>&) const {}
+  template <int W>
+  __device__ __forceinline__ Vec<W> tap(const Vec<W>& v, const K<W>&) const { return v; }
+};
+struct WinoBnRelu {
+  const float *__restrict__ mean, *__restrict__ invstd, *__restrict__ gamma, *__restrict__ beta;
+  template <int W>
+  struct K {
+    Vec<W> mu, is, ga, be;
+  };
+  template <int W>
+  __device__ __forceinline__ void load(int c, K<W>& k) const {
+    k.mu = vload<W>(mean + c), k.is = vload<W>(invstd + c), k.ga = vload<W>(gamma + c), k.be = vload<W>(beta + c);
+  }
+  template <int W>
+  __device__ __forceinline__ Vec<W> tap(const Vec<W>& v, const K<W>& k) const {
+    Vec<W> r;
+#pragma unroll
+    for (int q = 0; q < W; ++q) r.v[q] = fmaxf(pm_bn_affine(v.v[q], k.mu.v[q], k.is.v[q], k.ga.v[q], k.be.v[q]), 0.f);
+    return r;
+  }
+};
+
+template <int MT, int W, typename PRO>
+__global__ __launch_bounds__(256) void wino_input_kernel(const float* __restrict__ x, long xp, int C, int Kp, const pm_wino_geom g, float* __restrict__ V, const PRO pro) {
   constexpr int A = MT + 2;
   const unsigned kg = Kp / W;
   const unsigned total = (unsigned)g.tiles * kg;
@@ -119,6 +146,8 @@
     const int c = (int)(i - tile * kg) * W;
     const TileId t = decode_tile(tile, g);
     const bool cok = c < C;
+    typename PRO::template K<W> pk;
+    if (cok) pro.template load<W>(c, pk);
     Vec<W> tt[A][A];
 #pragma unroll
     for (int b = 0; b < A; ++b) {
@@ -128,7 +157,7 @@
 #pragma unroll
       for (int a = 0; a < A; ++a) {
         const int yy = t.ry + g.d * (MT * t.ty + a - 1);
-        col[a] = (xok && (unsigned)yy < (unsigned)g.H) ? vload<W>(x + ((long)(t.n * g.H + yy) * g.W + xx) * xp + c) : vzero<W>();
+        col[a] = (xok && (unsigned)yy < (unsigned)g.H) ? pro.template tap<W>(vload<W>(x + ((long)(t.n * g.H + yy) * g.W + xx) * xp + c), pk) : vzero<W>();
       }
       mat_apply<MT, W_BT>(col, o);
 #pragma unroll
@@ -311,6 +340,87 @@
   }
 }
 
+template <int MT, int W, bool ZOUT>
+__global__ __launch_bounds__(256) void wino_bn_bwd_kernel(const float* __restrict__ g, long gp, const float* __restrict__ y, long yp, int C, int Kp,
+                                                          const pm_wino_geom geo, const pm_wino_bn bn, float* __restrict__ V, float* __restrict__ Z, long zp) {
+  constexpr int A = MT + 2;
+  const unsigned kg = Kp / W;
+  const unsigned total = (unsigned)geo.tiles * kg;
+  const long vplane = geo.tiles * (long)Kp, zplane = geo.tiles * (long)C;
+  const float inv_n = bn.dev_count ? 1.f / bn.sums[2 * C] : bn.host_inv_n;
+  for (unsigned i = blockIdx.x * 256u + threadIdx.x; i < total; i += gridDim.x * 256u) {
+    const unsigned tile = i / kg;
+    const int c = (int)(i - tile * kg) * W;
+    float* vout = V + (long)tile * Kp + c;
+    if (c >= C) {
+#pragma unroll
+      for (int p = 0; p < A * A; ++p) vstore<W>(vout + p * vplane, vzero<W>());
+      continue;
+    }
+    const TileId t = decode_tile(tile, geo);
+    const Vec<W> mu = vload<W>(bn.mean + c), is = vload<W>(bn.invstd + c), ga = vload<W>(bn.gamma + c), be = vload<W>(bn.beta + c);
+    const Vec<W> s1 = vload<W>(bn.sums + c), s2 = vload<W>(bn.sums + C + c);
+    Vec<W> k2, sg;
+#pragma unroll
+    for (int q = 0; q < W; ++q) k2.v[q] = inv_n * s2.v[q], sg.v[q] = is.v[q] * ga.v[q];
+    Vec<W> tt[A][A], r[A][MT];
+#pragma unroll
+    for (int b = 0; b < A; ++b) {
+      const int xx = t.rx + geo.d * (MT * t.tx + b - 1);
+      const bool xok = (unsigned)xx < (unsigned)geo.W;
+      Vec<W> col[A], o[A];
+#pragma unroll
+      for (int a = 0; a < A; ++a) {
+        const int yy = t.ry + geo.d * (MT * t.ty + a - 1);
+        col[a] = vzero<W>();
+        if (xok && (unsigned)yy < (unsigned)geo.H) {
+          const long pix = (long)(t.n * geo.H + yy) * geo.W + xx;
+          const Vec<W> gv = vload<W>(g + pix * gp + c), yv = vload<W>(y + pix * yp + c);
+#pragma unroll
+          for (int q = 0; q < W; ++q) {
+            const float gm = pm_bn_affine(yv.v[q], mu.v[q], is.v[q], ga.v[q], be.v[q]) > 0.f ? gv.v[q] : 0.f;
+            float a1 = fmaf(-inv_n, s1.v[q], gm);
+            a1 = fmaf(-((yv.v[q] - mu.v[q]) * is.v[q]), k2.v[q], a1);
+            float dy = sg.v[q] * a1;
+            asm volatile("" : "+v"(dy));
+            col[a].v[q] = dy;
+          }
+          if constexpr (!ZOUT)
+            if (a >= 1 && a <= MT && b >= 1 && b <= MT) vstore<W>(Z + pix * zp + c, col[a]);
+        }
+      }
+      mat_apply<MT, W_BT>(col, o);
+#pragma unroll
+      for (int a = 0; a < A; ++a) tt[a][b] = o[a];
+      if (ZOUT && b >= 1 && b <= MT) {
+        Vec<W> in[MT];
+#pragma unroll
+        for (int a = 0; a < MT; ++a) in[a] = col[a + 1];
+        mat_apply<MT, W_A>(in, o);
+#pragma unroll
+        for (int a = 0; a < A; ++a) r[a][b - 1] = o[a];
+      }
+    }
+#pragma unroll
+    for (int a = 0; a < A; ++a) {
+      Vec<W> o[A];
+      mat_apply<MT, W_BT>(tt[a], o);
+#pragma unroll
+      for (int b = 0; b < A; ++b) vstore<W>(vout + (a * A + b) * vplane, o[b]);
+    }
+    if constexpr (ZOUT) {
+      float* zout = Z + (long)tile * C + c;
+#pragma unroll
+      for (int a = 0; a < A; ++a) {
+        Vec<W> o[A];
+        mat_apply<MT, W_A>(r[a], o);
+#pragma unroll
+        for (int b = 0; b < A; ++b) vstore<W>(zout + (a * A + b) * zplane, o[b]);
+      }
+    }
+  }
+}
+
 template <int MT>
 __global__ __launch_bounds__(256) void wino_dw_kernel(const float* __restrict__ slab, int ks, int Cout, int Cin, int Kp, float* __restrict__ dw) {
   constexpr int A = MT + 2, P = A * A;
@@ -506,9 +616,29 @@
 }
 
 int pm_wino_input_xf(const float* x, long pitch, int C, int Kp, const pm_wino_geom& g, float* V, hipStream_t st) {
-  if (g.m == 4) hipLaunchKernelGGL((wino_input_kernel<4, 2>), dim3(nblocks(g.tiles * (Kp / 2))), dim3(256), 0, st, x, pitch, C, Kp, g, V);
-  else hipLaunchKernelGGL((wino_input_kernel<2, 4>), dim3(nblocks(g.tiles * (Kp / 4))), dim3(256), 0, st, x, pitch, C, Kp, g, V);
+  if (g.m == 4) hipLaunchKernelGGL((wino_input_kernel<4, 2, WinoRaw>), dim3(nblocks(g.tiles * (Kp / 2))), dim3(256), 0, st, x, pitch, C, Kp, g, V, WinoRaw{});
+  else hipLaunchKernelGGL((wino_input_kernel<2, 4, WinoRaw>), dim3(nblocks(g.tiles * (Kp / 4))), dim3(256), 0, st, x, pitch, C, Kp, g, V, WinoRaw{});
   return pm_check_launch("wino_input");
+}
+
+int pm_wino_input_bn_xf(const float* x, long pitch, int C, int Kp, const pm_wino_geom& g, const pm_wino_bn& bn, float* V, hipStream_t st) {
+  const WinoBnRelu pro = {bn.mean, bn.invstd, bn.gamma, bn.beta};
+  if (g.m == 4) hipLaunchKernelGGL((wino_input_kernel<4, 2, WinoBnRelu>), dim3(nblocks(g.tiles * (Kp / 2))), dim3(256), 0, st, x, pitch, C, Kp, g, V, pro);
+  else hipLaunchKernelGGL((wino_input_kernel<2, 4, WinoBnRelu>), dim3(nblocks(g.tiles * (Kp / 4))), dim3(256), 0, st, x, pitch, C, Kp, g, V, pro);
+  return pm_check_launch("wino_input_bn");
+}
+
+int pm_wino_bn_bwd_xf(const float* g, long gpitch, const float* y, long ypitch, int C, int Kp, const pm_wino_geom& geo, const pm_wino_bn& bn, float* V, float* Z,
+                      float* dy, long dypitch, hipStream_t st) {
+  const dim3 grid(nblocks(geo.tiles * (Kp / (geo.m == 4 ? 2 : 4))));
+  if (Z) {
+    if (geo.m == 4) hipLaunchKernelGGL((wino_bn_bwd_kernel<4, 2, true>), grid, dim3(256), 0, st, g, gpitch, y, ypitch, C, Kp, geo, bn, V, Z, 0l);
+    else hipLaunchKernelGGL((wino_bn_bwd_kernel<2, 4, true>), grid, dim3(256), 0, st, g, gpitch, y, ypitch, C, Kp, geo, bn, V, Z, 0l);
+  } else {
+    if (geo.m == 4) hipLaunchKernelGGL((wino_bn_bwd_kernel<4, 2, false>), grid, dim3(256), 0, st, g, gpitch, y, ypitch, C, Kp, geo, bn, V, dy, dypitch);
+    else hipLaunchKernelGGL((wino_bn_bwd_kernel<2, 4, false>), grid, dim3(256), 0, st, g, gpitch, y, ypitch, C, Kp, geo, bn, V, dy, dypitch);
+  }
+  return pm_check_launch("wino_bn_bwd");
 }
 
 int pm_wino_filter_xf(const float* w, int Cout, int Cin, int Kp, bool dgrad, int m, float* U, hipStream_t st) {
diff --git a/pinthememory_amd/hip/kernels.py b/pinthememory_amd/hip/kernels.py
--- a/pinthememory_amd/hip/kernels.py
+++ b/pinthememory_amd/hip/kernels.py
@@ -234,7 +234,20 @@
     return _XFORM_COUNT[0]
 
 
-def conv_fwd(x, w_krsc, stride, pad, dil, bias=None, scale=None, shift=None, residual=None, relu=False, out=None, keep_v=None, bn_partials=None, out_dtype=None):
+def wino_z_bytes(x_shape, w_shape_krsc, stride, pad, dil, like):
+    cout, kh, kw, cin = w_shape_krsc
+    if not (KEEP_WINOGRAD_V and CONV_PREC == 0 and ACT_DTYPE == torch.float32 and like.dtype == torch.float32 and kh == 3 and kw == 3 and stride == 1):
+        return 0
+    n, h, w_, _ = x_shape
+
+    def ask():
+        xd, yd = L.PmTensor(256, n, h, w_, cin, cin, L.PM_F32, 0), L.PmTensor(256, n, h, w_, cout, cout, L.PM_F32, 0)
+        return _lib().pm_conv_winograd_z_bytes(byref(xd), byref(yd), byref(L.conv_params(kh, kw, stride, pad, dil, CONV_PREC)))
+    return _sizes(('z', tuple(x_shape), tuple(w_shape_krsc), stride, pad, dil, CONV_PREC, _GEN[0]), ask)
+
+
+def conv_fwd(x, w_krsc, stride, pad, dil, bias=None, scale=None, shift=None, residual=None, relu=False, out=None, keep_v=None, bn_partials=None, out_dtype=None,
+             in_bn=None):
     cout, kh, kw, cin = w_krsc.shape
     n, h, w_, c = x.shape
     assert c == cin, 'conv: Cin mismatch %d vs %d' % (c, cin)
@@ -271,7 +284,12 @@
         rd = tdesc(residual) if residual is not None else None
         ep = L.conv_epilogue(ptr(bias), ptr(scale), ptr(shift), rd.ptr if rd else None, rd.pitch if rd else 0, 1 if relu else 0, ptr(part),
                             part.numel() * 4 if part is not None else 0)
-    check(lib.pm_conv_fwd(byref(xd), w_krsc.data_ptr(), byref(yd), byref(p), byref(ep) if ep else None, ptr(ws), nb, stream()), 'pm_conv_fwd')
+    if in_bn is not None:
+        assert x.dtype == torch.float32 and y.dtype == torch.float32, 'conv_fwd(in_bn=...): fp32 tier only'
+        check(lib.pm_conv_fwd_bn(xd.ptr, xd.pitch, n, h, w_, c, *[t.data_ptr() for t in in_bn], w_krsc.data_ptr(), yd.ptr, yd.pitch, cout, byref(p), byref(ep) if ep else None,
+                                 ptr(ws), nb, stream()), 'pm_conv_fwd_bn')
+    else:
+        check(lib.pm_conv_fwd(byref(xd), w_krsc.data_ptr(), byref(yd), byref(p), byref(ep) if ep else None, ptr(ws), nb, stream()), 'pm_conv_fwd')
     if u_ent is not None:
         _U_CACHE.commit(u_ent)
     return y
@@ -297,7 +315,29 @@
     return dx
 
 
-def conv_bwd_weight(x, dy, w_shape_krsc, stride, pad, dil, want_bias=False, wino_v=None, on_stream=None):
+def conv_bwd_data_bn(g, y, mean, invstd, gamma, beta, sums, count, w_krsc, x_shape, stride, pad, dil, add=None, z_event=None):
+    cout, kh, kw, cin = w_krsc.shape
+    dx = new(x_shape, g)
+    gd, yd, dxd = tdesc(g), tdesc(y), tdesc(dx)
+    p = L.conv_params(kh, kw, stride, pad, dil, CONV_PREC)
+    lib = _lib()
+    nb = _sizes(('d', g.shape, g.stride(), g.dtype, gd.flags, w_krsc.shape, dx.shape, dx.stride(), dx.dtype, stride, pad, dil, CONV_PREC, _GEN[0]),
+                lambda: (lib.pm_conv_workspace(byref(dxd), byref(gd), byref(p), 1), lib.pm_conv_wxf_bytes_dgrad(byref(gd), byref(dxd), byref(p))))[0]
+    nbz = wino_z_bytes(x_shape, tuple(w_krsc.shape), stride, pad, dil, g)
+    z = torch.empty(nbz // 4, dtype=torch.float32, device=g.device) if nbz else None
+    dy = None if nbz else torch.empty(g.shape, dtype=torch.float32, device=g.device)
+    dyd = tdesc(dy) if dy is not None else None
+    ws = workspace(nb, g.device) if nb else None
+    ad = tdesc(add) if add is not None else None
+    assert g.dtype == y.dtype == dx.dtype == torch.float32 and tuple(g.shape) == tuple(y.shape) and (add is None or tuple(add.shape) == tuple(dx.shape))
+    check(lib.pm_conv_bwd_data_bn(gd.ptr, gd.pitch, yd.ptr, yd.pitch, gd.n, gd.h, gd.w, cout, mean.data_ptr(), invstd.data_ptr(), gamma.data_ptr(), beta.data_ptr(),
+                                  sums.data_ptr(), float(count), w_krsc.data_ptr(), dxd.ptr, dxd.pitch, cin, byref(p), ad.ptr if ad else None, ad.pitch if ad else 0,
+                                  ptr(z), nbz, dyd.ptr if dyd else None, dyd.pitch if dyd else 0, z_event.cuda_event if z_event is not None else None, ptr(ws), nb,
+                                  stream()), 'pm_conv_bwd_data_bn')
+    return dx, z, dy
+
+
+def conv_bwd_weight(x, dy, w_shape_krsc, stride, pad, dil, want_bias=False, wino_v=None, on_stream=None, z=None):
     cout, kh, kw, cin = w_shape_krsc
     dw = torch.empty(w_shape_krsc, dtype=torch.float32, device=x.device)
     db = torch.empty(cout, dtype=torch.float32, device=x.device) if want_bias else None
@@ -310,7 +350,12 @@
                 lambda: lib.pm_conv_workspace(byref(xd), byref(dyd), byref(p), 2))
     raw = stream() if on_stream is None else on_stream.cuda_stream
     ws = workspace(nb, x.device, on_stream)
-    check(lib.pm_conv_bwd_weight(byref(xd), byref(dyd), dw.data_ptr(), ptr(db), byref(p), ptr(ws), nb, raw), 'pm_conv_bwd_weight')
+    if z is not None:
+        assert not want_bias
+        check(lib.pm_conv_bwd_weight_z(xd.ptr, xd.pitch, xd.n, xd.h, xd.w, cin, cout, z.data_ptr(), z.numel() * 4, dw.data_ptr(), byref(p), ptr(ws), nb, raw),
+              'pm_conv_bwd_weight_z')
+    else:
+        check(lib.pm_conv_bwd_weight(byref(xd), byref(dyd), dw.data_ptr(), ptr(db), byref(p), ptr(ws), nb, raw), 'pm_conv_bwd_weight')
     return dw, db
 
 
diff --git a/pinthememory_amd/hip/lib.py b/pinthememory_amd/hip/lib.py
--- a/pinthememory_amd/hip/lib.py
+++ b/pinthememory_amd/hip/lib.py
@@ -94,6 +94,11 @@
     'pm_conv_bwd_data': (_i, [_T, _vp, _T, _P, _T, _vp, _sz, _vp]),
     'pm_conv_bwd_data_masked': (_i, [_T, _vp, _T, _P, _T, _vp, _vp, _sz, _vp]),
     'pm_conv_bwd_weight': (_i, [_T, _T, _vp, _vp, _P, _vp, _sz, _vp]),
+    'pm_conv_winograd_z_bytes': (_sz, [_T, _T, _P]),
+    'pm_conv_fwd_bn': (_i, [_vp, _i64, _i, _i, _i, _i, _vp, _vp, _vp, _vp, _vp, _vp, _i64, _i, _P, _E, _vp, _sz, _vp]),
+    'pm_conv_bwd_data_bn': (_i, [_vp, _i64, _vp, _i64, _i, _i, _i, _i, _vp, _vp, _vp, _vp, _vp, _f, _vp, _vp, _i64, _i, _P, _vp, _i64, _vp, _sz, _vp, _i64, _vp, _vp, _sz,
+                                 _vp]),
+    'pm_conv_bwd_weight_z': (_i, [_vp, _i64, _i, _i, _i, _i, _i, _vp, _sz, _vp, _P, _vp, _sz, _vp]),
     'pm_set_winograd': (_i, [_i]),
     'pm_set_winograd_fused': (_i, [_i]),
     'pm_set_conv16': (_i, [_i]),
diff --git a/pinthememory_amd/hip/ops.py b/pinthememory_amd/hip/ops.py
--- a/pinthememory_amd/hip/ops.py
+++ b/pinthememory_amd/hip/ops.py
@@ -130,16 +130,20 @@
     return (p, True) if p is not None else (weight, False)
 
 
-def _wgrad(x, dy, wshape, geom, want_bias=False, deferred=False, wino_v=None):
+def _wgrad(x, dy, wshape, geom, want_bias=False, deferred=False, wino_v=None, z=None, after=None):
     if not deferred:
-        return K.conv_bwd_weight(x, dy, wshape, *geom, want_bias=want_bias, wino_v=wino_v)
+        return K.conv_bwd_weight(x, dy, wshape, *geom, want_bias=want_bias, wino_v=wino_v, z=z)
     side, main = _side_stream(), L.stream_obj()
-    ev = torch.cuda.Event()
-    ev.record(main)
+    ev = after
+    if ev is None:
+        ev = torch.cuda.Event()
+        ev.record(main)
     side.wait_event(ev)
-    out = K.conv_bwd_weight(x, dy, wshape, *geom, want_bias=want_bias, wino_v=wino_v, on_stream=side)
+    out = K.conv_bwd_weight(x, dy, wshape, *geom, want_bias=want_bias, wino_v=wino_v, on_stream=side, z=z)
     if wino_v is not None:
         wino_v.record_stream(side)
+    if z is not None:
+        z.record_stream(side)
     x.record_stream(side)
     dy.record_stream(side)
     for t in out:
@@ -239,6 +243,27 @@
     return (K.bn_bwd_apply_mask(dv, mask, y, mean, invstd, gamma, S.total(0), S.count(y)), *S.grads(0))
 
 
+def _wino_bn_ok(x_shape, w_shape_krsc, geom, like):
+    return K.wino_z_bytes(tuple(x_shape), tuple(w_shape_krsc), *geom, like) != 0
+
+
+def _bn_conv_bwd(dv, y, mean, invstd, gamma, beta, group, wk, x, geom, vk, deferred, want_dx=True):
+    if not (want_dx and vk is not None and _wino_bn_ok(x.shape, wk.shape, geom, dv)):
+        dy, _, dgamma, dbeta = _bn_train_bwd(dv, None, y, mean, invstd, gamma, beta, True, group, False, False)
+        dw, _ = _wgrad(x, dy, tuple(wk.shape), geom, deferred=deferred, wino_v=vk)
+        return (K.conv_bwd_data(dy, wk, tuple(x.shape), *geom, dtype=x.dtype) if want_dx else None), dw, dgamma, dbeta
+    S = _BnSums(1, y.shape[3], group, y.device)
+    K.bn_bwd_reduce(dv, None, y, mean, invstd, 2, gamma, beta, want_gmask=False, with_count=S.with_count, sums=S.slot(0))
+    S.exchange()
+    ev = None
+    if deferred:
+        ev = torch.cuda.Event()
+        ev.record(L.stream_obj())
+    dx, z, _ = K.conv_bwd_data_bn(dv, y, mean, invstd, gamma, beta, S.total(0), S.count(y), wk, tuple(x.shape), *geom, z_event=ev)
+    dw, _ = _wgrad(x, y, tuple(wk.shape), geom, deferred=deferred, wino_v=vk, z=z, after=ev)
+    return (dx, dw, *S.grads(0))
+
+
 class _Bottleneck(torch.autograd.Function):
 
     @staticmethod
@@ -247,9 +272,13 @@
         k1, k2, k3 = K.krsc(w1), K.krsc(w2), K.krsc(w3)
         ps = []
         y1 = K.conv_fwd(xv, k1, *geoms[0], bn_partials=ps)
-        o1, m1, i1 = _bn_train_fwd(y1, g1, b1, bns[0], None, True, partials=ps[0])
         kv = []
-        y2 = K.conv_fwd(o1, k2, *geoms[1], keep_v=kv, bn_partials=ps)
+        if y1.dtype == torch.float32 and _wino_bn_ok(y1.shape, k2.shape, geoms[1], y1):
+            (m1, i1), o1 = _bn_train_stats(y1, bns[0], ps[0]), None
+            y2 = K.conv_fwd(y1, k2, *geoms[1], keep_v=kv, bn_partials=ps, in_bn=(m1, i1, g1, b1))
+        else:
+            o1, m1, i1 = _bn_train_fwd(y1, g1, b1, bns[0], None, True, partials=ps[0])
+            y2 = K.conv_fwd(o1, k2, *geoms[1], keep_v=kv, bn_partials=ps)
         o2, m2, i2 = _bn_train_fwd(y2, g2, b2, bns[1], None, True, partials=ps[1])
         y3 = K.conv_fwd(o2, k3, *geoms[2], bn_partials=ps)
         m3 = None
@@ -296,9 +325,7 @@
             dy3, dres, dg3, db3 = _bn_train_bwd(dv, out, y3, m3, i3, g3, b3, True, gr[2], True, True, mask=mask3)
         dw3, _ = _wgrad(o2, dy3, tuple(k3.shape), ge[2], deferred=df[2])
         do2 = K.conv_bwd_data(dy3, k3, tuple(o2.shape), *ge[2])
-        dy2, _, dg2, db2 = _bn_train_bwd(do2, o2, y2, m2, i2, g2, b2, True, gr[1], False, False)
-        dw2, _ = _wgrad(o1, dy2, tuple(k2.shape), ge[1], deferred=df[1], wino_v=v2)
-        do1 = K.conv_bwd_data(dy2, k2, tuple(o1.shape), *ge[1])
+        do1, dw2, dg2, db2 = _bn_conv_bwd(do2, y2, m2, i2, g2, b2, gr[1], k2, o1 if o1 is not None else y1, ge[1], v2, df[1])
         dy1, _, dg1, db1 = _bn_train_bwd(do1, o1, y1, m1, i1, g1, b1, True, gr[0], False, False)
         dw1, _ = _wgrad(xv, dy1, tuple(k1.shape), ge[0], deferred=df[0])
         dwd = dgd = dbd = None
@@ -403,6 +430,10 @@
         stride, pad, dil = ctx.geom
         dv = _grad_view(dout)
         want_dres = ctx.has_res and ctx.needs_input_grad[5]
+        if (ctx.train and ctx.relu and not ctx.has_res and not ctx.has_bias and ctx.needs_input_grad[0] and ctx.needs_input_grad[1] and vk is not None
+                and dv.dtype == torch.float32 and _wino_bn_ok(xv.shape, wk.shape, ctx.geom, dv)):
+            dx, dwk, dgamma, dbeta = _bn_conv_bwd(dv, y, mean, invstd, gamma, beta, ctx.group, wk, xv, ctx.geom, vk, ctx.deferred)
+            return nchw(dx), dwk.permute(0, 3, 1, 2), None, dgamma, dbeta, None, None, None, None, None, None
         if ctx.train:
             dy, dres, dgamma, dbeta = _bn_train_bwd(dv, o, y, mean, invstd, gamma, beta, ctx.relu, ctx.group, want_dres, ctx.has_res)
         else:
@@ -418,6 +449,30 @@
             dwk, db = _wgrad(xv, dy, tuple(wk.shape), (stride, pad, dil), want_bias=ctx.has_bias, deferred=ctx.deferred, wino_v=vk)
             dw = dwk.permute(0, 3, 1, 2)
         return dx, dw, db, dgamma, dbeta, (nchw(dres) if dres is not None else None), None, None, None, None, None
+
+
+class _ConvBnActPair(torch.autograd.Function):
+
+    @staticmethod
+    def forward(ctx, x, wa, ga, ba, wb, gb, bb, geoms, bns, deferred):
+        xv, ka, kb = nhwc(x), K.krsc(wa), K.krsc(wb)
+        kva, kvb, ps = [], [], []
+        ya = K.conv_fwd(xv, ka, *geoms[0], keep_v=kva, bn_partials=ps)
+        ma, ia = _bn_train_stats(ya, bns[0], ps[0])
+        yb = K.conv_fwd(ya, kb, *geoms[1], keep_v=kvb, bn_partials=ps, in_bn=(ma, ia, ga, ba))
+        ob, mb, ib = _bn_train_fwd(yb, gb, bb, bns[1], None, True, partials=ps[1])
+        ctx.geoms, ctx.groups, ctx.deferred = geoms, [b.group for b in bns], deferred
+        ctx.save_for_backward(xv, ka, kb, ya, yb, ma, ia, mb, ib, ga, ba, gb, bb, kva[0], kvb[0])
+        return nchw(ob)
+
+    @staticmethod
+    def backward(ctx, dout):
+        xv, ka, kb, ya, yb, ma, ia, mb, ib, ga, ba, gb, bb, va, vb = ctx.saved_tensors
+        ge, gr, df = ctx.geoms, ctx.groups, ctx.deferred
+        doa, dwb, dgb, dbb = _bn_conv_bwd(_grad_view(dout), yb, mb, ib, gb, bb, gr[1], kb, ya, ge[1], vb, df[1])
+        dx, dwa, dga, dba = _bn_conv_bwd(doa, ya, ma, ia, ga, ba, gr[0], ka, xv, ge[0], va, df[0], ctx.needs_input_grad[0])
+        p = lambda d: d.permute(0, 3, 1, 2)
+        return (nchw(dx) if dx is not None else None), p(dwa), dga, dba, p(dwb), dgb, dbb, None, None, None
 
 
 class _Stem(torch.autograd.Function):
@@ -729,6 +784,18 @@
     return _ConvBnAct.apply(x, w, conv.bias, bn.weight, bn.bias, residual, _geom(conv), BNState(bn), relu, out, deferred)
 
 
+def conv_bn_act_pair(x, conv_a, bn_a, conv_b, bn_b):
+    n, _, h, w = x.shape
+    ga, gb = _geom(conv_a), _geom(conv_b)
+    ha, wa_ = K.conv_out_hw(h, w, conv_a.kernel_size[0], *ga)
+    wb_shape = (conv_b.out_channels, conv_b.kernel_size[0], conv_b.kernel_size[1], conv_b.in_channels)
+    if (torch.is_grad_enabled() and bn_a.training and bn_b.training and conv_a.bias is None and conv_b.bias is None and x.dtype == torch.float32
+            and conv_a.weight.requires_grad and conv_b.weight.requires_grad and _wino_bn_ok((n, ha, wa_, conv_b.in_channels), wb_shape, gb, x)):
+        (wa, da), (wb, db) = _w(conv_a.weight), _w(conv_b.weight)
+        return _ConvBnActPair.apply(x, wa, bn_a.weight, bn_a.bias, wb, bn_b.weight, bn_b.bias, [ga, gb], [BNState(bn_a), BNState(bn_b)], [da, db])
+    return conv_bn_act(conv_bn_act(x, conv_a, bn_a, relu=True), conv_b, bn_b, relu=True)
+
+
 def bottleneck(x, blk):
     ds = blk.downsample
     mods = [(blk.conv1, blk.bn1), (blk.conv2, blk.bn2), (blk.conv3, blk.bn3)] + ([(ds[0], ds[1])] if ds is not None else [])
diff --git a/pinthememory_amd/network/deepv3plus.py b/pinthememory_amd/network/deepv3plus.py
--- a/pinthememory_amd/network/deepv3plus.py
+++ b/pinthememory_amd/network/deepv3plus.py
@@ -218,8 +218,7 @@
         dec0_fine = run_cbr(self.bot_fine, low_level, out=buf[:, :48])
         dec0_up = ops.resize(dec0_up, low_level.size()[2:], out=buf[:, 48:])
         dec0 = ops.concat(buf, [dec0_fine, dec0_up])
-        dec1 = ops.conv_bn_act(dec0, self.final1[0], self.final1[1], relu=True)
-        dec1 = ops.conv_bn_act(dec1, self.final1[3], self.final1[4], relu=True)
+        dec1 = ops.conv_bn_act_pair(dec0, self.final1[0], self.final1[1], self.final1[3], self.final1[4])
         dec2 = ops.conv(dec1, self.final2[0])
         return self._finish(dec2, x_size, aux_out, gts, aux_gts, mem_output, writeloss, readloss, inter_feature)
 
```

Result: no change. 159.1 (-0.5%).
